# edavalosanaya/FastPoseCNN

Measured on AMD Instinct MI355X. Metric: img/s end-to-end 640x480 inference; hough-vote kernel HBM GB/s vs roofline, higher is better.
Workload: dtype f32

## Files before the change

fastposecnn_amd/_native.py:

```python
import ctypes
import os

import torch

_HERE = os.path.dirname(os.path.abspath(__file__))
LIB_PATH = os.path.join(_HERE, "libfpc_hip.so")

_lib = None

_vp = ctypes.c_void_p
_i = ctypes.c_int
_i64 = ctypes.c_int64
_u64 = ctypes.c_uint64
_f = ctypes.c_float
_d = ctypes.c_double
_sz = ctypes.c_size_t

_SIGNATURES = {
    "fpc_abi_version": (ctypes.c_int, []),
    "fpc_error_string": (ctypes.c_char_p, [_i]),
    "fpc_last_hip_error": (ctypes.c_char_p, []),
    "fpc_generate_hypothesis": (_i, [_vp, _vp, _vp, _vp, _i, _i, _i, _vp]),
    "fpc_voting_for_hypothesis": (_i, [_vp, _vp, _vp, _vp, _i, _i, _i, _f, _vp]),
    "fpc_ransac_workspace_bytes": (_sz, [_i, _i, _i, _i]),
    "fpc_ransac_voting_v3": (_i, [_vp, _vp, _i64, _i64, _i64, _i64, _i, _vp, _i, _i, _i, _vp, _vp, _u64, _f, _i, _i,
                                  _vp, _vp, _vp, _vp, _vp, _vp, _vp, _vp, _vp, _sz, _vp]),
    "fpc_ransac_voting_v3_bits": (_i, [_vp, _vp, _vp, _i64, _i64, _i64, _i64, _i, _vp, _i, _i, _i, _vp, _vp, _u64, _f, _i, _i, _vp, _vp, _vp, _vp, _vp, _vp, _vp, _vp, _vp, _sz, _vp]),
    "fpc_ransac_voting_v3_pose": (_i, [_vp, _vp, _vp, _i64, _i64, _i64, _i64, _i, _vp, _i, _i, _i, _vp, _vp, _u64, _f, _i, _i, _vp, _vp, _vp, _vp, _vp, _vp, _vp, _vp,
                                       _vp, _vp, _vp, _vp, _vp, _vp, _vp, _sz, _vp]),
    "fpc_vote_set_prune": (_i, [_i, _i, ctypes.POINTER(ctypes.c_int32)]),
    "fpc_vote_prune_info": (_i, [_vp, _sz, _i, _i, _i, _i, _vp, _vp]),
    "fpc_class_compress": (_i, [_vp, _vp, _vp, _vp, _vp, _vp, _i, _i, _i, _vp, _vp, _vp, _vp, _vp, _vp]),
    "fpc_class_compress_bits": (_i, [_vp, _vp, _vp, _vp, _vp, _vp, _i, _i, _i, _vp, _vp, _vp, _vp, _vp, _vp, _vp]),
    "fpc_cc_workspace_bytes": (_sz, [_i, _i, _i]),
    "fpc_cc_bits_supported": (_i, [_i, _i, _i]),
    "fpc_fg_bits": (_i, [_vp, _i, _i, _i, _vp, _vp]),
    "fpc_cc_label_bits": (_i, [_vp, _i, _i, _i, _vp, _vp, _vp, _i, _vp, _sz, _vp]),
    "fpc_cc_label": (_i, [_vp, _i, _i, _i, _vp, _vp, _vp, _i, _vp, _sz, _vp]),
    "fpc_aggregate_workspace_bytes": (_sz, [_i]),
    "fpc_aggregate": (_i, [_vp, _vp, _vp, _vp, _vp, _vp, _i, _i, _i, _i, _vp, _vp, _vp, _vp, _vp, _vp, _vp, _vp, _vp, _vp, _sz,
                           _vp]),
    "fpc_aggregate_bits": (_i, [_vp, _vp, _vp, _vp, _vp, _vp, _i, _i, _i, _i, _vp, _vp, _vp, _vp, _vp, _vp, _vp, _vp, _vp, _vp, _vp, _vp, _sz, _vp]),
    "fpc_mask_bits_words": (_sz, [_i, _i]),
    "fpc_pose_errors": (_i, [_vp, _vp, _vp, _vp, _i, _vp, _vp, _vp, _vp, _vp, _vp, _i, _vp, _vp, _vp, _vp]),
    "fpc_pose_metrics_state_words": (_sz, [_i, _i, _i, _i, _i]),
    "fpc_pose_metrics_update": (_i, [_vp, _vp, _vp, _i, _i] + [_vp] * 11 + [_i, _vp, _i, _vp, _i, _vp, _i, _vp, _i, _vp, _i] + [_vp] * 5 + [_i, _vp]),
    "fpc_confusion_update": (_i, [_vp, _vp, _i64, _i, _vp, _vp]),
    "fpc_post_network_backward": (_i, [_vp, _vp, _i, _i, _i, _i, _vp, _vp, _f, _i, _u64, _vp, _vp, _vp, _vp, _vp, _vp]),
    "fpc_vote_refine_backward": (_i, [_vp, _vp, _i64, _i64, _i64, _i64, _i, _i, _i, _vp, _f, _i, _u64, _vp, _vp, _vp]),
    "fpc_class_compress_backward": (_i, [_vp, _vp, _vp, _vp, _vp, _vp, _vp, _i, _i, _i, _vp, _vp, _vp, _vp, _vp]),
    "fpc_mask_losses": (_i, [_vp, _vp, _i, _i, _i, _i64, _i64, _f, _f, _vp, _vp, _vp, _vp]),
    "fpc_match_assign": (_i, [_vp, _vp, _vp, _i, _i, _vp, _vp, _vp, _vp]),
    "fpc_matched_losses": (_i, [_vp, _vp, _vp, _i, _i] + [_vp] * 10 + [_i, _d, _i, _i, _i, ctypes.POINTER(_d)] + [_vp] * 5),
    "fpc_matched_losses_backward": (_i, [_vp, _vp, _vp, _i, _i] + [_vp] * 10 + [_i, _d, _i, _i, _i, ctypes.POINTER(_d)] + [_vp] * 8),
    "fpc_grad_sumsq": (_i, [_vp, _sz, _vp, _vp]),
    "fpc_lookahead_radam_step": (_i, [_vp, _vp, _vp, _vp, _vp, _sz, _f, _f, _f, _f, _f, _i64, _i, _f, _vp, _vp]),
    "fpc_pose_rt": (_i, [_vp, _vp, _vp, _vp, _i, _vp, _vp, _vp, _vp]),
    "fpc_pack_pose_records": (_i, [_vp] * 9 + [_i, _i, _i, _vp, _vp]),
    "fpc_mask_iou_workspace_bytes": (_sz, [_i, _i, _i64]),
    "fpc_mask_iou": (_i, [_vp, _i, _vp, _i, _i64, _i, _vp, _vp, _vp, _vp, _sz, _vp]),
    "fpc_preprocess_workspace_bytes": (_sz, [_i]),
    "fpc_preprocess_u8": (_i, [_vp, _i, _i, _i, ctypes.POINTER(ctypes.c_double), ctypes.POINTER(ctypes.c_double), _i, _vp, _vp,
                               _sz, _vp]),
    "fpc_png_info": (_i, [_vp, _sz, ctypes.POINTER(ctypes.c_int32)]),
    "fpc_png_decode": (_i, [_vp, _sz, _vp, _sz, _i]),
    "fpc_png_decode_batch": (_i, [ctypes.POINTER(_vp), ctypes.POINTER(_sz), _i, _vp, _i, _i, _i]),
    "fpc_gt_build": (_i, [_vp, _i64, _i64, _i, _i, _i, _vp, _vp, _vp, _i, _vp, _vp, _i, _vp, _vp]),
    "fpc_depth_decode": (_i, [_vp, _i, _i, _i, _i, _i, _vp, _vp]),
    "fpc_net_create": (_i, [ctypes.c_char_p, _i, _i, _i, _i, ctypes.POINTER(_vp)]),
    "fpc_net_create_encoder": (_i, [_i, ctypes.POINTER(_i), _i, _i, _i, _i, ctypes.POINTER(_vp)]),
    "fpc_net_destroy": (None, [_vp]),
    "fpc_net_set_graph": (_i, [_vp, _i]),
    "fpc_net_set_split_precision": (_i, [_vp, _i]),
    "fpc_net_param_count": (_i, [_vp]),
    "fpc_net_param_name": (ctypes.c_char_p, [_vp, _i]),
    "fpc_net_param_numel": (_i64, [_vp, _i]),
    "fpc_net_workspace_bytes": (_sz, [_vp]),
    "fpc_net_load_params": (_i, [_vp, _vp, _i, _vp, _sz, _vp]),
    "fpc_net_forward": (_i, [_vp, _vp, _vp, _vp, _vp, _vp, _vp, _vp, _vp, _vp, _vp, _vp, _vp]),
    "fpc_net_forward_bits": (_i, [_vp, _vp, _vp, _vp, _vp, _vp, _vp, _vp, _vp, _vp, _vp, _vp, _vp, _vp]),
    "fpc_net_autotune_next": (_i, [_vp, _i]),
    "fpc_net_conv_count": (_i, [_vp]),
    "fpc_net_conv_plan": (_i, [_vp, _i, ctypes.POINTER(_i)]),
    "fpc_net_copy_plans": (_i, [_vp, _vp]),
    "fpc_net_force_winograd": (_i, [_vp, _i]),
    "fpc_net_force_pointwise": (_i, [_vp, _i]),
    "fpc_net_force_fold": (_i, [_vp, _i]),
    "fpc_net_force_direct_h3": (_i, [_vp, _i]),
    "fpc_net_force_stem_pool": (_i, [_vp, _i]),
    "fpc_act_range": (_i, [_vp, ctypes.c_longlong, _vp, _vp]),
    "fpc_net_survey_next": (_i, [_vp, _vp, _i]),
    "fpc_net_guard_ranges": (_i, [_vp, ctypes.POINTER(ctypes.c_uint32), _i, _f, _f]),
    "fpc_net_guarded": (_i, [_vp, _i]),
    "fpc_stem_pool_tasks": (_i, [_i, _i, ctypes.POINTER(_i64)]),
    "fpc_wino_pack_geometry": (_i, [_i, _i, _i, _i, _i, ctypes.POINTER(_i64)]),
    "fpc_net_set_wino_pack": (_i, [_vp, _i]),
    "fpc_net_set_wino_orient": (_i, [_vp, _i]),
    "fpc_wino_orient_geometry": (_i, [_i, _i, _i, _i, _i, _i, ctypes.POINTER(_i64)]),
    "fpc_net_wino_blocks": (_i64, [_vp]),
    "fpc_net_graph_recorded": (_i, [_vp]),
    "fpc_net_flops": (_i, [_vp, ctypes.POINTER(ctypes.c_double)]),
    "fpc_net_tensor": (_i, [_vp, ctypes.c_char_p, ctypes.POINTER(_vp), ctypes.POINTER(_i), ctypes.POINTER(_i),
                            ctypes.POINTER(_i)]),
    "fpc_conv2d_workspace_bytes": (_sz, [_i, _i, _i, _i, _i, _i, _i]),
    "fpc_conv2d_workspace_bytes_for": (_sz, [_i, _i, _i, _i, _i, _i, _i, _i, _i, _i]),
    "fpc_conv2d_plan": (_i, [_i, _i, _i, _i, _i, _i, _i, _i, _i, _i, ctypes.POINTER(_i)]),
    "fpc_conv2d": (_i, [_vp, _i64, _i64, _i64, _i64, _vp, _vp, _vp, _vp, _vp, _vp, _vp, _i, _i, _i, _i, _i, _i, _i, _i,
                        _i, _i, _i, _i, _i, _vp, _sz, _vp]),
    "fpc_conv2d_wgrad_workspace_bytes": (_sz, [_i, _i, _i, _i, _i, _i, _i]),
    "fpc_upsample_bilinear_fwd": (_i, [_vp, _i64, _i64, _i64, _i64, _vp, _i, _i, _i, _i, _i, _i, _vp]),
    "fpc_upsample_bilinear_bwd_scratch_floats": (_sz, [_i, _i, _i, _i, _i]),
    "fpc_upsample_bilinear_bwd": (_i, [_vp, _i64, _i64, _i64, _i64, _vp, _vp, _i, _i, _i, _i, _i, _i, _vp]),
    "fpc_groupnorm4_relu_scratch_floats": (_sz, [_i, _i, _i]),
    "fpc_groupnorm4_relu_fwd": (_i, [_vp, _vp, _vp, _vp, _vp, _vp, _i, _i, _i, _i, ctypes.c_float, _vp]),
    "fpc_groupnorm4_relu_bwd": (_i, [_vp, _vp, _vp, _vp, _vp, _vp, _vp, _i, _i, _i, _i, _vp]),
    "fpc_batchnorm_scratch_floats": (_sz, [_i, _i]),
    "fpc_batchnorm_fwd": (_i, [_vp, _vp, _vp, _vp, _vp, _vp, _vp, _vp, _vp, _i, _i, _f, _f, _i, _vp]),
    "fpc_batchnorm_bwd": (_i, [_vp, _vp, _vp, _vp, _vp, _vp, _vp, _vp, _vp, _vp, _i, _i, _i, _vp]),
    "fpc_conv2d_wgrad": (_i, [_vp, _i64, _i64, _i64, _vp, _vp, _i, _i, _i, _i, _i, _i, _i, _i, _i, _vp, _sz, _vp]),
    "fpc_conv2d_wgrad_split": (_i, [_vp, _i64, _i64, _i64, _vp, _vp, _i, _i, _i, _i, _i, _i, _i, _i, _i, _vp, _sz, _vp]),
}

EXPORTED = tuple(_SIGNATURES)


def lib():
    global _lib
    if _lib is None:
        if not os.path.exists(LIB_PATH):
            raise RuntimeError(
                f"fastposecnn_amd: {LIB_PATH} is missing — build it with `python -m fastposecnn_amd.build` "
                "(hipcc --offload-arch=gfx950). There is no CPU fallback for the HIP hot path.")
        L = ctypes.CDLL(LIB_PATH)
        for name, (res, args) in _SIGNATURES.items():
            fn = getattr(L, name)
            fn.restype = res
            fn.argtypes = args
        if L.fpc_abi_version() != 11:
            raise RuntimeError("fastposecnn_amd: libfpc_hip.so ABI version mismatch")
        _lib = L
    return _lib


def check(rc, what):
    if rc != 0:
        L = lib()
        msg = L.fpc_error_string(rc).decode()
        hip = L.fpc_last_hip_error().decode() if rc == -3 else ""
        raise RuntimeError(f"fastposecnn_amd: {what} failed: {msg} (code {rc}){' — HIP: ' + hip if hip else ''}")


def ptr(t):
    return None if t is None else t.data_ptr()


_raw_stream = getattr(torch._C, "_cuda_getCurrentRawStream", None)
_cur_device = getattr(torch._C, "_cuda_getDevice", None)


def stream():
    if _raw_stream is not None and _cur_device is not None:
        return _raw_stream(_cur_device())
    return torch.cuda.current_stream().cuda_stream


def require_gpu(*tensors, what="this op"):
    for t in tensors:
        if t is not None and not t.is_cuda:
            raise RuntimeError(f"fastposecnn_amd: {what} runs only on GPU tensors (HIP kernels, no CPU fallback)")


_workspaces = {}


def workspace(tag, device, nbytes):
    key = (tag, device.index, stream())
    ws = _workspaces.get(key)
    if ws is None or ws.numel() < nbytes:
        ws = torch.empty(max(int(nbytes), 256), dtype=torch.uint8, device=device)
        assert ws.data_ptr() % 256 == 0
        _workspaces[key] = ws
    return ws
```

fastposecnn_amd/csrc/net.hip:

```cpp
#include <math.h>
#include <stdio.h>
#include <stdlib.h>
#include <string.h>

#include <initializer_list>
#include <string>
#include <utility>
#include <vector>

#include "net_kernels.hpp"

namespace fpc {

struct PackedConv {
    int Cin = 0, Cinp = 0, Cout = 0, Kh = 1, Kw = 1, stride = 1, pad = 0;
    int Kwp = 1;
    int K = 0, Kpad = 0, Npad = 0;
    int p_w = -1;
    int p_bn = -1;
    int p_bias = -1;
    size_t w_off = 0, scale_off = 0, shift_off = 0;
    size_t wino_off = 0;
    bool wino_ok = false;
    size_t h3_off = 0;
// ... 1118 lines not shown
                        float* logits_xy, float* logits_z, int64_t* cat_mask, float* cq, float* cs, float* cxy, float* cz,
                        uint64_t* fg_bits, fpc_stream_t stream);

extern "C" int fpc_net_forward_bits(fpc_net_t* n, const float* x, float* logits_mask, float* logits_quat,
                                    float* logits_scales, float* logits_xy, float* logits_z, int64_t* cat_mask, float* cq,
                                    float* cs, float* cxy, float* cz, uint64_t* fg_bits, fpc_stream_t stream) {
    const int rc = forward_bits(n, x, logits_mask, logits_quat, logits_scales, logits_xy, logits_z, cat_mask, cq, cs, cxy, cz, fg_bits, stream);
    if (n) n->survey = nullptr;
    return rc;
}

static int forward_bits(fpc_net_t* n, const float* x, float* logits_mask, float* logits_quat, float* logits_scales,
                        float* logits_xy, float* logits_z, int64_t* cat_mask, float* cq, float* cs, float* cxy, float* cz,
                        uint64_t* fg_bits, fpc_stream_t stream) {
    if (!n || !n->loaded || !x || !cat_mask || !cq || !cs || !cxy || !cz) return FPC_EINVAL;
    if (fg_bits && (n->W % 64 != 0 || ((uintptr_t)fg_bits & 7))) return FPC_EINVAL;
    bool any = logits_mask || logits_quat || logits_scales || logits_xy || logits_z;
    bool all = logits_mask && logits_quat && logits_scales && logits_xy && logits_z;
    if (any && !all) return FPC_EINVAL;
    hipStream_t s = (hipStream_t)stream;
    float* ws = n->ws;
    const int B = n->B, H = n->H, W = n->W;

    FPC_TRY(launch_nchw3_to_nhwc4(x, ws + n->a_img4.off, B, H * W, s));
    const bool plain = n->tuning || n->survey;
    if (n->use_graph && !plain && s != nullptr && !n->graph_exec) {
        hipGraph_t g = nullptr;
        if (hipStreamBeginCapture(s, hipStreamCaptureModeThreadLocal) == hipSuccess) {
            int rc = forward_middle(n, s);
            hipError_t e = hipStreamEndCapture(s, &g);
            if (rc) { if (g) (void)hipGraphDestroy(g); return rc; }
            if (e == hipSuccess && g) e = hipGraphInstantiate(&n->graph_exec, g, nullptr, nullptr, 0);
            if (g) (void)hipGraphDestroy(g);
            if (e != hipSuccess) n->graph_exec = nullptr;
        }
        if (!n->graph_exec) { (void)hipGetLastError(); n->use_graph = 0; }
    }
    if (n->use_graph && !plain && s != nullptr && n->graph_exec) {
        if (hipGraphLaunch(n->graph_exec, s) != hipSuccess) return FPC_ELAUNCH;
    } else {
        FPC_TRY(forward_middle(n, s));
    }
    {
        Up4Args u;
        memset(&u, 0, sizeof(u));
        u.lm = ws + n->a_low[0].off; u.lq = ws + n->a_low[1].off; u.lt = ws + n->a_low[2].off; u.ls = ws + n->a_low[3].off;
        u.pm = n->dec[0].head_chp; u.pq = n->dec[1].head_chp; u.pt = n->dec[2].head_chp; u.ps = n->dec[3].head_chp;
        u.o_mask = logits_mask; u.o_quat = logits_quat; u.o_scales = logits_scales; u.o_xy = logits_xy; u.o_z = logits_z;
        u.cat_mask = (long long*)cat_mask; u.cq = cq; u.cs = cs; u.cxy = cxy; u.cz = cz;
        u.B = B; u.hl = n->a_low[0].H; u.wl = n->a_low[0].W; u.H = H; u.W = W; u.C = n->classes;
        u.fg_bits = reinterpret_cast<unsigned long long*>(fg_bits); u.fg_stride = (size_t)((H * W + 4095) / 4096) * 64;
        if (u.hl * 4 != H || u.wl * 4 != W) return FPC_EINVAL;
        FPC_TRY(launch_up4_compress(u, s));
    }
    if (n->tuning) { n->tuning = false; n->tuned = true; }
    return FPC_OK;
}

extern "C" int fpc_net_autotune_next(fpc_net_t* n, int mode) {
    if (!n || !n->loaded || mode < 0 || mode > 2) return FPC_EINVAL;
    n->tuning = true;
    n->tune_mode = mode;
    drop_graph(n);
    return FPC_OK;
}

extern "C" int fpc_net_survey_next(fpc_net_t* n, unsigned* records_dev, int sites) {
    if (n && !records_dev) { n->survey = nullptr; return FPC_OK; }
    if (!n || !n->loaded || ((uintptr_t)records_dev & 3) || sites != (int)n->convs.size()) return FPC_EINVAL;
    n->survey = records_dev;
    return FPC_OK;
}

static ConvPlan range_free_plan(const fpc_net* n, int i) {
    if (n->has_free[i]) return n->free_plan[i];
    const PackedConv& c = n->convs[i];
    ConvPlan q = n->cplan[i];
    if (q.pool) { ConvPlan st; st.stem = 256; return st; }
    if (q.wino) {
        q.wino = wino_form_ok(kWinoW4, c.Cin, c.Cout) ? kWinoW4 : kWinoBf3;
        q.fold = 0;
        return q;
    }
    q.h3 = 0; q.bf3 = 1;
    return q;
}

extern "C" int fpc_net_guard_ranges(fpc_net_t* n, const unsigned* records_host, int sites, float lo, float hi) {
    if (!n || !records_host || sites != (int)n->convs.size() || !(lo >= 0.f) || !(hi > lo)) return FPC_EINVAL;
    auto outside = [&](int site) {
        const unsigned* rec = records_host + 4 * (size_t)site;
        float mx;
        memcpy(&mx, &rec[0], sizeof(mx));
        return rec[2] != 0 && (rec[1] > 0 || mx >= hi || (mx > 0.f && mx < lo));
    };
    int demoted = 0;
    for (int i = 0; i < sites; ++i) {
        if (!n->c_groups[i] || !plan_range_limited(n->cplan[i]) || records_host[4 * (size_t)i + 2] == 0) continue;
        if (!(outside(i) || (n->cplan[i].fold && outside(n->dec[0].lat[3])))) continue;
        n->cplan[i] = range_free_plan(n, i);
        n->guarded[i] = 1;
        ++demoted;
    }
    if (demoted) drop_graph(n);
    return demoted;
}

extern "C" int fpc_net_guarded(const fpc_net_t* n, int i) {
    return n && i >= 0 && i < (int)n->guarded.size() && n->guarded[i] ? 1 : 0;
}

extern "C" int fpc_net_conv_count(const fpc_net_t* n) { return n ? (int)n->convs.size() : 0; }
extern "C" int fpc_net_conv_plan(const fpc_net_t* n, int i, int* out5) {
    if (!n || !out5 || i < 0 || i >= (int)n->convs.size()) return FPC_EINVAL;
    const ConvPlan& p = n->cplan[i];
    out5[0] = p.bm; out5[1] = p.bn;
    if (p.lat) { out5[0] = 128; out5[1] = 32; }
    if (p.stem) { out5[0] = 64; out5[1] = 64; }
    if (p.pw) { out5[0] = pw_tile_pixels(p.pw - 1); out5[1] = 64; }
    out5[2] = encode_plan(p, n->fold_ok && i == n->dec[0].lat[3] && n->cplan[n->dec[0].seg[6]].fold);
    out5[3] = n->convs[i].Cout; out5[4] = n->convs[i].K;
    return FPC_OK;
}

extern "C" int fpc_net_force_winograd(fpc_net_t* n, int form) {
    if (!n || form < 1 || form >= kWinoFormCount) return FPC_EINVAL;
    int changed = 0;
    for (size_t i = 0; i < n->convs.size(); ++i) {
        const PackedConv& c = n->convs[i];
        if (!c.wino_ok || !n->c_groups[i] || !wino_form_ok(form, c.Cin, c.Cout)) continue;
        ConvPlan q = n->cplan[i];
        q.wino = form; q.lat = 0; q.stem = 0;
        if (form != kWinoH3) q.fold = 0;
        n->cplan[i] = q;
        n->guarded[i] = 0;
        ++changed;
    }
    drop_graph(n);
    return changed;
}

extern "C" int fpc_net_force_fold(fpc_net_t* n, int on) {
    if (!n || on < 0 || on > 1 || (on && !n->fold_ok)) return FPC_EINVAL;
    ConvPlan& p = n->cplan[n->dec[0].seg[6]];
    if (p.fold == on) return 0;
    ConvPlan q;
    q.wino = kWinoH3; q.fold = on;
    p = q;
    n->guarded[n->dec[0].seg[6]] = 0;
    drop_graph(n);
    return 1;
}

extern "C" int fpc_net_force_pointwise(fpc_net_t* n, int on) {
    if (!n || on < 0 || on > 1) return FPC_EINVAL;
    int changed = 0;
    for (size_t i = 0; i < n->convs.size(); ++i) {
        const PackedConv& c = n->convs[i];
        if (!n->c_groups[i] || c.Kh != 1 || c.pad != 0 || c.Cinp != c.Cin || c.Cin % 64 || c.Kpad != c.Cin || c.Cout % 64) continue;
        if (on) {
            if (n->cplan[i].pw) continue;
            ConvPlan q;
            q.pw = 1;
            n->cplan[i] = q;
        } else {
            if (!n->cplan[i].pw) continue;
            n->cplan[i] = plan_conv(n->c_howo[i], n->B, c.Cout, c.Kpad / kConvBK, n->c_groups[i]);
        }
        ++changed;
    }
    drop_graph(n);
    return changed;
}

extern "C" int fpc_net_force_direct_h3(fpc_net_t* n, int on) {
    if (!n || on < 0 || on > 1 || (on && !n->h3_packed)) return FPC_EINVAL;
    int changed = 0;
    for (size_t i = 0; i < n->convs.size(); ++i) {
        const PackedConv& c = n->convs[i];
        if (!c.h3_ok || !n->c_groups[i] || on == n->cplan[i].h3) continue;
        const ConvPlan& p = n->cplan[i];
        ConvPlan q = plan_conv(n->c_howo[i], n->B, c.Cout, c.Kpad / kConvBK, n->c_groups[i]);
        if (on && !p.wino && !p.stem && !p.pw) q = p;
        q.bf3 = 0;
        q.h3 = on;
        n->cplan[i] = q;
        n->guarded[i] = 0;
        ++changed;
    }
    drop_graph(n);
    return changed;
}

extern "C" int fpc_net_force_stem_pool(fpc_net_t* n, int on) {
    if (!n || on < 0 || on > 1 || (on && !n->h3_packed)) return FPC_EINVAL;
    if (on && ((n->a_stem.H & 1) || (n->a_stem.W & 63) || (long long)n->H * n->W * 16 >= (1LL << 31))) return FPC_EINVAL;
    ConvPlan& p = n->cplan[n->c_stem];
    if (p.pool == on) return 0;
    ConvPlan q;
    q.stem = 256; q.pool = on;
    p = q;
    n->guarded[n->c_stem] = 0;
    drop_graph(n);
    return 1;
}

extern "C" int fpc_net_copy_plans(fpc_net_t* dst, const fpc_net_t* src) {
    if (!dst || !src || dst->convs.size() != src->convs.size() || dst->H != src->H || dst->W != src->W) return FPC_EINVAL;
    for (size_t i = 0; i < dst->convs.size(); ++i) {
        const PackedConv &a = dst->convs[i], &b = src->convs[i];
        if (a.Cin != b.Cin || a.Cout != b.Cout || a.Kh != b.Kh || a.Kw != b.Kw || a.stride != b.stride || a.Npad != b.Npad ||
            a.Kpad != b.Kpad || dst->c_groups[i] != src->c_groups[i])
            return FPC_EINVAL;
    }
    for (size_t i = 0; i < dst->convs.size(); ++i) {
        const ConvPlan& q = src->cplan[i];
        if (splitk_floats_for(q, dst->c_groups[i] ? dst->c_groups[i] : 1, dst->B, dst->convs[i].Npad) > dst->splitk_floats) continue;
        if (q.nsplit > 1 && q.fused && !can_fuse(q, dst->c_groups[i] ? dst->c_groups[i] : 1, dst->B)) continue;
        if ((q.h3 || q.pool) && !dst->h3_packed) continue;
        dst->cplan[i] = q;
    }
    for (size_t i = 0; i < dst->convs.size(); ++i) {
        const ConvPlan& q = src->free_plan[i];
        const int groups = dst->c_groups[i] ? dst->c_groups[i] : 1;
        dst->has_free[i] = src->has_free[i] && splitk_floats_for(q, groups, dst->B, dst->convs[i].Npad) <= dst->splitk_floats &&
                           !(q.nsplit > 1 && q.fused && !can_fuse(q, groups, dst->B));
        if (dst->has_free[i]) dst->free_plan[i] = q;
        dst->guarded[i] = dst->guarded[i] || src->guarded[i];
        if (dst->guarded[i] && plan_range_limited(dst->cplan[i])) dst->cplan[i] = range_free_plan(dst, (int)i);
    }
    dst->tuned = true;
    drop_graph(dst);
    return FPC_OK;
}

extern "C" int fpc_net_flops(const fpc_net_t* n, double* out3) {
    if (!n || !out3) return FPC_EINVAL;
    double direct = 0.0, executed = 0.0, wino = 0.0;
    for (size_t i = 0; i < n->convs.size(); ++i) {
        if (!n->c_groups[i]) continue;
        const PackedConv& c = n->convs[i];
        const double f = 2.0 * n->B * (double)n->c_howo[i] * c.Cout * c.Cin * c.Kh * c.Kw * n->c_groups[i];
        direct += f;
        if (n->cplan[i].wino) { executed += f / 2.25; wino += f; } else executed += f;
    }
    for (int d = 0; d < 4; ++d)
        direct += 2.0 * n->B * (double)n->a_low[d].H * n->a_low[d].W * 128.0 * n->dec[d].head_ch,
        executed += 2.0 * n->B * (double)n->a_low[d].H * n->a_low[d].W * 128.0 * n->dec[d].head_ch;
    out3[0] = direct; out3[1] = executed; out3[2] = direct > 0.0 ? wino / direct : 0.0;
    return FPC_OK;
}

extern "C" int fpc_net_tensor(const fpc_net_t* n, const char* name, const float** ptr, int* H, int* W, int* C) {
    if (!n || !n->ws || !name || !ptr || !H || !W || !C) return FPC_EINVAL;
    Act t;
    bool ok = false;
    if (!strcmp(name, "stem")) {
        if (n->cplan[n->c_stem].pool) return FPC_EINVAL;
        t = n->a_stem; ok = true;
    }
    else if (!strcmp(name, "pool")) { t = n->a_pool; ok = true; }
    else if (name[0] == 'c' && name[1] >= '2' && name[1] <= '5' && !name[2]) { t = n->a_blk_y[name[1] - '2'].back(); ok = true; }
    else if (name[0] == 'd' && name[1] >= '0' && name[1] <= '3' && name[2] == '.') {
        int d = name[1] - '0';
        const char* r = name + 3;
        if (r[0] == 'p' && r[1] >= '2' && r[1] <= '5' && !r[2]) {
            if (r[1] == '2' && n->cplan[n->dec[0].seg[6]].fold) return FPC_EINVAL;
            t = n->a_p[d]['5' - r[1]]; ok = true;
        }
        else if (!strncmp(r, "seg", 3) && r[3] >= '0' && r[3] <= '6' && !r[4]) { t = n->a_seg[d][r[3] - '0']; ok = true; }
        else if (!strcmp(r, "low")) { t = n->a_low[d]; ok = true; }
    }
    if (!ok) return FPC_EINVAL;
    *ptr = n->ws + t.off; *H = t.H; *W = t.W; *C = t.C;
    return FPC_OK;
}

extern "C" int fpc_stem_pool_tasks(int Ho, int Wo, int64_t* out4) {
    if (!out4 || Ho < 2 || (Ho & 1) || Wo < 64 || (Wo & 63)) return FPC_EINVAL;
    long long o[4];
    stem_pool_tasks(Ho, Wo, kStemPoolBand, o);
    for (int i = 0; i < 4; ++i) out4[i] = o[i];
    return FPC_OK;
}

extern "C" int fpc_wino_pack_geometry(int H, int W, int B, int Cin, int fold, int64_t* out8) {
    if (!out8 || H < 1 || W < 1 || B < 1 || Cin < 1) return FPC_EINVAL;
    const WinoPackGeom q = wino_pack_geometry(H, W, B, Cin, !fold);
    out8[0] = q.G; out8[1] = q.tbx; out8[2] = q.tby; out8[3] = q.patches; out8[4] = q.slots; out8[5] = q.tiles; out8[6] = q.gn_rows;
    out8[7] = q.rx;
    return FPC_OK;
}

extern "C" int fpc_wino_orient_geometry(int H, int W, int B, int Cin, int fold, int pack, int64_t* out9) {
    if (!out9 || H < 1 || W < 1 || B < 1 || Cin < 1) return FPC_EINVAL;
    bool tr;
    const WinoPackGeom q = wino_launch_geometry(H, W, B, Cin, true, pack && !fold, &tr);
    out9[0] = tr ? 1 : 0;
    out9[1] = q.G; out9[2] = q.tbx; out9[3] = q.tby; out9[4] = q.patches; out9[5] = q.slots; out9[6] = q.tiles; out9[7] = q.gn_rows;
    out9[8] = q.rx;
    return FPC_OK;
}

extern "C" size_t fpc_conv2d_workspace_bytes(int B, int Ho, int Wo, int Cin, int Cout, int Kh, int Kw) {
    int K = Cin * Kh * Kw, Kpad = cdiv(K, kConvBK) * kConvBK, Npad = cdiv(Cout, kConvNAlign) * kConvNAlign;
    size_t packed = conv_packed_floats(Npad, Kpad);
    size_t splitk = (size_t)32 * B * (cdiv(Ho * Wo, 128) * 128) * Npad;
    size_t wino = wino_region_floats(kImgH3, Cout, Cin, true);
    return (packed + splitk + wino + kConvTickets) * sizeof(float);
}

namespace {
struct Conv2dLayout { size_t packed, splitk, wino, tickets, total; };
Conv2dLayout conv2d_layout(int B, int Cin, int Cout, int Kh, int Kw, const ConvPlan& p, const Conv2dRequest& r) {
    const int K = Cin * Kh * Kw, Kpad = cdiv(K, kConvBK) * kConvBK, Npad = cdiv(Cout, kConvNAlign) * kConvNAlign;
    Conv2dLayout L;
    L.packed = r.wino ? 0 : conv_packed_floats(Npad, Kpad);
    L.splitk = r.wino ? 0 : (splitk_floats_for(p, 1, B, Npad) + 63) / 64 * 64;
    L.wino = r.wino ? wino_region_floats(kWinoForms[r.wino].image, Cout, Cin, Cout % 128 == 0) : 0;
    L.tickets = (!r.wino && p.fused && p.nsplit > 1) ? kConvTickets : 0;
    L.total = L.packed + L.splitk + L.wino + L.tickets;
    return L;
}
ConvPlan conv2d_plan_for(int B, int Ho, int Wo, int Cin, int Cout, int Kh, int Kw, int bm, int bn, const Conv2dRequest& r) {
    const int Kpad = cdiv(Cin * Kh * Kw, kConvBK) * kConvBK;
    ConvPlan p = plan_conv(Ho * Wo, B, Cout, Kpad / kConvBK, 1, r.wino ? 0 : bm, bn, r.wino ? 1 : r.nsplit);
    p.bf3 = r.bf3 ? 1 : 0;
    p.h3 = r.h3 ? 1 : 0;
    if (r.two_launch) p.fused = 0;
    p.lat = r.lat;
    p.stem = r.stem ? 256 : 0;
    p.pool = r.pool ? 1 : 0;
    p.pw = r.pw;
    p.wino = r.wino;
    return p;
}
}

extern "C" int fpc_conv2d_plan(int B, int Ho, int Wo, int Cin, int Cout, int Kh, int Kw, int bm, int bn, int nsplit,
                               int* out4) {
    if (!out4) return FPC_EINVAL;
    const int Kpad = cdiv(Cin * Kh * Kw, kConvBK) * kConvBK;
    const Conv2dRequest r = decode_plan(nsplit);
    ConvPlan p = plan_conv(Ho * Wo, B, Cout, Kpad / kConvBK, 1, bm, bn, r.nsplit);
    p.wino = r.wino;
    out4[0] = p.bm; out4[1] = p.bn; out4[2] = r.wino ? nsplit : p.nsplit; out4[3] = plan_gn_rows(p, Ho, Wo, B, Cin, r.pack, r.orient);
    return FPC_OK;
}

extern "C" size_t fpc_conv2d_workspace_bytes_for(int B, int Ho, int Wo, int Cin, int Cout, int Kh, int Kw, int bm, int bn,
                                                 int nsplit) {
    if (B < 1 || Ho < 1 || Wo < 1 || Cin < 1 || Cout < 1 || Kh < 1 || Kw < 1) return 0;
    const Conv2dRequest r = decode_plan(nsplit);
    const ConvPlan p = conv2d_plan_for(B, Ho, Wo, Cin, Cout, Kh, Kw, bm, bn, r);
    return std::max<size_t>(conv2d_layout(B, Cin, Cout, Kh, Kw, p, r).total * sizeof(float), 256);
}

extern "C" int fpc_conv2d(const float* in, int64_t sb, int64_t sh, int64_t sw, int64_t sc, const float* w_oihw,
                          const float* scale, const float* shift, const float* res, const float* up, float* out,
                          float* gn_part, int B, int Hi, int Wi, int Cin, int Cout, int Kh, int Kw, int stride, int pad,
                          int relu, int bm, int bn, int nsplit, void* ws, size_t ws_bytes, fpc_stream_t stream) {
    if (!in || !w_oihw || !out || !ws || B < 1 || Kh != Kw) return FPC_EINVAL;
    int Ho = conv_out(Hi, Kh, stride, pad), Wo = conv_out(Wi, Kw, stride, pad);
    if (Ho < 1 || Wo < 1) return FPC_EINVAL;
    const Conv2dRequest rq = decode_plan(nsplit);
    const int wino = rq.wino;
    ConvPlan p = conv2d_plan_for(B, Ho, Wo, Cin, Cout, Kh, Kw, bm, bn, rq);
    const Conv2dLayout lay = conv2d_layout(B, Cin, Cout, Kh, Kw, p, rq);
    if (ws_bytes < lay.total * sizeof(float) || ((uintptr_t)ws & 255)) return FPC_EWORKSPACE;
    PackedConv c;
    c.Cin = c.Cinp = Cin; c.Cout = Cout; c.Kh = Kh; c.Kw = Kw; c.stride = stride; c.pad = pad;
    c.K = Cin * Kh * Kw; c.Kpad = cdiv(c.K, kConvBK) * kConvBK; c.Npad = cdiv(Cout, kConvNAlign) * kConvNAlign;
    hipStream_t s = (hipStream_t)stream;
    float* packed = (float*)ws;
    if (rq.stem) {
        if (Cin != 4 || Kh != 7 || stride != 2 || pad != 3 || Cout != 64 || sc != 1 || sw != 4 || sh != (int64_t)4 * Wi ||
            sb != (int64_t)4 * Hi * Wi || res || up || gn_part)
            return FPC_EINVAL;
        c.Kwp = 8; c.K = 4 * 7 * 8; c.Kpad = 224;
        FPC_TRY((rq.pool ? launch_pack_weight_h3 : launch_pack_weight_bf3)(w_oihw, packed, Cout, Cin, Cin, Kh, Kw, c.Kwp, c.Npad, c.Kpad, s));
        fpc_net tmp0;
        tmp0.B = B; tmp0.ws = packed; tmp0.splitk_off = lay.packed;
        ConvArgs a0;
        fill_conv_args(&tmp0, a0, c, p, Hi, Wi, Ho, Wo, sb, sh, sw, sc, relu != 0, 0);
        a0.Cin = 8 * c.Cinp; a0.Kw = 1; a0.K = c.K; a0.lanepx = 1;
        a0.p[0] = ConvPtrs{in, packed, out, scale, shift, nullptr, nullptr, nullptr};
        return rq.pool ? launch_stem_pool(a0, packed, out, Ho / 2, Wo / 2, s) : launch_conv_plan(a0, p, 1, s);
    }
    static_assert(FPC_IGEMM_DMA_B, "the split-precision direct form stages its B rows from the bf16 planes by LDS-DMA; a build that loads "
                                   "them from the f32 image must pack that image here as well");
    if (!wino) FPC_TRY((p.h3 ? launch_pack_weight_h3 : p.bf3 ? launch_pack_weight_bf3 : launch_pack_weight)(w_oihw, packed, Cout, Cin, Cin, Kh, Kw, Kw, c.Npad, c.Kpad, s));
    int mode = (sc == 1 && Cin % kConvBK == 0 && Kh * Kw <= 32 && ((int64_t)Hi + 2 * pad) * sh * 4 < ((int64_t)1 << 31)) ? 0
               : (sc == 1 && Cin % 4 == 0 && sw % 4 == 0 && sh % 4 == 0 && sb % 4 == 0 && ((uintptr_t)in & 15) == 0) ? 2 : 1;
    fpc_net tmp;
    tmp.B = B;
    tmp.wino_pack = rq.pack ? 1 : 0;
    tmp.wino_orient = rq.orient ? 1 : 0;
    tmp.ws = packed;
    tmp.splitk_off = lay.packed;
    ConvArgs a;
    fill_conv_args(&tmp, a, c, p, Hi, Wi, Ho, Wo, sb, sh, sw, sc, relu != 0, mode);
    a.p[0] = ConvPtrs{in, packed, out, scale, shift, res, up, gn_part};
    a.zeros = nullptr;
    a.tickets = nullptr;
    if (lay.tickets) {
        float* tk = packed + lay.packed + lay.splitk + lay.wino;
        a.tickets = (int*)tk;
        if (hipMemsetAsync(tk, 0, kConvTickets * sizeof(int), s) != hipSuccess) return FPC_ELAUNCH;
    }
#ifdef FPC_STAMP_WINO
    if (wino && relu == 77) { a.dbg = gn_part; a.p[0].gn_part = nullptr; a.relu = 0; }
#endif
#ifdef FPC_STAMP_IGEMM
    if (!wino && relu == 77) { a.dbg = gn_part; a.p[0].gn_part = nullptr; a.relu = 0; }
#endif
    if (wino) {
        if (Kh != 3 || stride != 1 || pad != 1 || Cin % 8 || Cout % 64 || sc != 1 || up || sw != Cin ||
            sh != (int64_t)Wi * Cin || sb != (int64_t)Hi * Wi * Cin)
            return FPC_EINVAL;
        float* wp = packed + lay.packed + lay.splitk;
        if (!wino_form_ok(wino, Cin, Cout)) return FPC_EINVAL;
        const WinoImage img = kWinoForms[wino].image;
        if (rq.orient && wino_orient_rule(Ho, Wo)) FPC_TRY(launch_wino_pack_h3(w_oihw, wp + wino_image_offset(img, Cout, Cin), Cout, Cin, true, s));
        else FPC_TRY(kWinoImages[img].pack(w_oihw, wp + wino_image_offset(img, Cout, Cin), Cout, Cin, s));
        a.wino_w[0] = wp;
        a.zeros = zero_page();
        if (!a.zeros) {
            float* zp = wp + lay.wino - 64;
            if (hipMemsetAsync(zp, 0, 64 * sizeof(float), s) != hipSuccess) return FPC_ELAUNCH;
            a.zeros = zp;
        }
        return launch_conv_plan(a, p, 1, s);
    }
    if (p.h3) {
        if (mode != 0) return FPC_EINVAL;
        a.h3_w[0] = packed;
        return launch_conv_plan(a, p, 1, s);
    }
    a.bf3 = (p.bf3 && mode == 0) ? 1 : 0;
    if (p.bf3 && mode != 0) return FPC_EINVAL;
    if (p.lat || p.pw) return launch_conv_plan(a, p, 1, s);
    return run_conv(nullptr, a, 1, 0, s);
}
```

fastposecnn_amd/csrc/net_kernels.hpp:

```cpp
#pragma once
#include "common.hpp"

namespace fpc {

#ifndef FPC_IGEMM_DMA_B
#define FPC_IGEMM_DMA_B 1
#endif

constexpr int kMaxGroup = 4;
constexpr int kConvBK = 32;
constexpr int kConvNAlign = 128;
constexpr int kConvTickets = 16384;

struct ConvPtrs {
    const float* in;
    const float* w;
    float* out;
    const float* scale;
    const float* shift;
    const float* res;
    const float* up;
    float* gn_part;
};

struct ConvArgs {
    ConvPtrs p[kMaxGroup];
    float* splitk_ws;
    int* tickets;
    int fused;
    int B, Hi, Wi, Cin, Ho, Wo, Cout, Npad, Kh, Kw, stride, pad, K, Kpad;
    long long in_sb, in_sh, in_sw, in_sc;
    int relu, nsplit, mtiles, ntiles, ksteps, bm, bn, generic, groups;
    int bf3;
    int h3;
    int lanepx;
    const float* wino_w[kMaxGroup];
    const float* h3_w[kMaxGroup];
    const float* zeros;
    const float* fold_in;
    const float* fold_w[kMaxGroup];
    const float* fold_w2[kMaxGroup];
    const float* fold_up[kMaxGroup];
    const float* fold_tab[kMaxGroup];
    int fold_cin;
    float fold_lat_ms;
    void* dbg;
    long long wino_blocks;
    int wino_pack;
    int wino_orient;
};

struct LatArgs {
    const float* in;
    const unsigned short* wpl[kMaxGroup];
    float* out[kMaxGroup];
    const float* shift[kMaxGroup];
    const float* up[kMaxGroup];
    int B, Ho, Wo, Cout, Npad, Kpad, groups, relu;
    unsigned bias_mask;
    int parts;
    int h3;
};
int launch_lateral1x1(const LatArgs& a, hipStream_t s);

struct PwArgs {
    const float* in;
    const unsigned short* wpl[kMaxGroup];
    float* out[kMaxGroup];
    const float* scale[kMaxGroup];
    const float* shift[kMaxGroup];
    const float* res[kMaxGroup];
    const float* up[kMaxGroup];
    long long in_sb, in_sh, in_sw;
    int B, Ho, Wo, Cin, Cout, Npad, Kpad, stride, groups, relu;
    int has_scale, has_shift, has_res, has_up;
    int variant;
};
int launch_conv1x1(const PwArgs& a, hipStream_t s);
inline int pw_tile_pixels(int variant) { return variant == 0 ? 64 : 128; }

struct StemArgs {
    const float* in;
    const unsigned short* wpl;
    float* out;
    const float* scale;
    const float* shift;
    int B, Hi, Wi, Ho, Wo, Cout, Npad, Kpad, relu;
    int grid;
};
int launch_stem7x7(const StemArgs& a, hipStream_t s);

struct StemPoolArgs {
    const float* in;
    const unsigned short* wpl;
    float* out;
    const float* scale;
    const float* shift;
    int B, Hi, Wi, Ho, Wo, Hp, Wp, Npad, Kpad, relu;
    int band;
    int grid;
};
constexpr int kStemPoolBand = 10;
int launch_stem_pool_h3(const StemPoolArgs& a, hipStream_t s);
void stem_pool_tasks(int Ho, int Wo, int band, long long out4[4]);

constexpr int kMaxGnSites = 4;
struct GnFinArgs {
    const float* gn_part[kMaxGnSites * kMaxGroup];
    const float* gamma[kMaxGnSites * kMaxGroup];
    const float* beta[kMaxGnSites * kMaxGroup];
    float* affine[kMaxGnSites * kMaxGroup];
    int P[kMaxGnSites];
    long long count[kMaxGnSites];
    int B, C, groups, sites;
    float eps;
};

constexpr int kMaxUpJobs = 2;
struct GnUpArgs {
    const float* in[kMaxUpJobs * kMaxGroup];
    const float* affine[kMaxUpJobs * kMaxGroup];
    float* out[kMaxUpJobs * kMaxGroup];
    int h[kMaxUpJobs], w[kMaxUpJobs];
    int B, C, jobs;
};

struct MergeHeadArgs {
    const float* t_lo[kMaxGroup][3];
    const float* a_lo[kMaxGroup][3];
    const float* t_hi[kMaxGroup];
    const float* a_hi[kMaxGroup];
    const float* hw[kMaxGroup];
    const float* hb[kMaxGroup];
    float* out[kMaxGroup];
    int ch[kMaxGroup];
    int chp[kMaxGroup];
    int B, h, w, C;
};

struct HeadPartArgs {
    const float* t[kMaxGroup][3];
    const float* aff[kMaxGroup][3];
    const float* hw[kMaxGroup];
    const float* hb[kMaxGroup];
    const float* lsum[kMaxGroup];
    float* out[kMaxGroup];
    int ch[kMaxGroup], chp[kMaxGroup];
    int B, H, W, C, hl, wl;
};
int launch_head_part(const HeadPartArgs& a, bool hi, int groups, hipStream_t s);

struct Up4Args {
    const float* lm; const float* lq; const float* lt; const float* ls;
    int pm, pq, pt, ps;
    float* o_mask; float* o_quat; float* o_scales; float* o_xy; float* o_z;
    long long* cat_mask; float* cq; float* cs; float* cxy; float* cz;
    int B, hl, wl, H, W, C;
    unsigned long long* fg_bits; size_t fg_stride;
};

#ifdef FPC_STAMP_WINO
constexpr bool kWinoStamp = true;
#else
constexpr bool kWinoStamp = false;
#endif

struct WinoArgs {
    ConvPtrs p[kMaxGroup];
    long long* dbg;
    const float* zeros;
    int variant;
    int groups;
    int waves;
    int B, H, W, Cin, Cout, relu, tbx, tby;
    const float* in2[kMaxGroup];
    const float* w2[kMaxGroup];
    const float* btab[kMaxGroup];
    int fold, Cin2;
    int pack, pack_rx;
    int orient;
};
int launch_conv_wino(const WinoArgs& a, int groups, hipStream_t s);
const float* zero_page();
int launch_wino_pack(const float* w_oihw, float* packed, int Cout, int Cin, hipStream_t s);
int launch_wino_pack_bf3(const float* w_oihw, float* packed, int Cout, int Cin, hipStream_t s);
int launch_conv_wino_c128(const WinoArgs& a, int groups, hipStream_t s);
int launch_wino_pack_c128(const float* w_oihw, float* packed, int Cout, int Cin, hipStream_t s);
int launch_conv_wino_w4(const WinoArgs& a, int groups, hipStream_t s);
int launch_conv_wino_h2(const WinoArgs& a, int groups, hipStream_t s);
int launch_wino_pack_h2(const float* w_oihw, float* packed, int Cout, int Cin, hipStream_t s);
int launch_absmax_bits(const float* w, long long n, unsigned* out_bits, hipStream_t s);
int launch_act_range(const float* x, long long n, unsigned* rec4, hipStream_t s);
int launch_conv_wino_h3(const WinoArgs& a, int groups, hipStream_t s);
struct WinoPackGeom { int G, tbx, tby, rx; long long patches, slots, tiles; int gn_rows; };
WinoPackGeom wino_pack_geometry(int H, int W, int B, int Cin, bool allow);
bool wino_orient_rule(int H, int W);
WinoPackGeom wino_launch_geometry(int H, int W, int B, int Cin, bool orient, bool pack_allow, bool* transposed);
int launch_wino_pack_h3(const float* w_oihw, float* packed, int Cout, int Cin, bool transpose, hipStream_t s);
int launch_wino_pack_h3_pair(const float* w1, float* packed1, int Cin1, const float* w2, float* packed2, int Cin2, int Cout, bool transpose,
                             hipStream_t s);
int launch_fold_compose(const float* W, const float* L, const float* bias, float* wc, float* btab, int Cout, int Cmid, int Cin,
                        bool transpose, hipStream_t s);
int launch_conv(const ConvArgs& a, int groups, hipStream_t s);
int launch_conv_splitk_epilogue(const ConvArgs& a, int groups, hipStream_t s);
int launch_maxpool3x3s2(const float* in, float* out, int B, int Hi, int Wi, int C, int Ho, int Wo, hipStream_t s);
int launch_gn_finalize(const GnFinArgs& a, int groups, hipStream_t s);
int launch_gn_relu_up2(const GnUpArgs& a, int groups, hipStream_t s);
int launch_merge_head(const MergeHeadArgs& a, int groups, hipStream_t s);
int launch_up4_compress(const Up4Args& a, hipStream_t s);
void launch_up4_compress7x4(const Up4Args& a, hipStream_t s);

struct Lerp { int i0, i1; float l0, l1; };
__device__ __forceinline__ Lerp lerp_coord(int dst, int in, int out) {
    float scale = out > 1 ? (float)(in - 1) / (float)(out - 1) : 0.f;
    float src = scale * (float)dst;
    Lerp L;
    L.i0 = (int)src;
    L.i1 = L.i0 + (L.i0 < in - 1 ? 1 : 0);
    L.l1 = src - (float)L.i0;
    L.l0 = 1.f - L.l1;
    return L;
}

__device__ __forceinline__ Lerp lerp_scaled(int dst, int in, float scale) {
    float src = scale * (float)dst;
    Lerp L;
    L.i0 = (int)src;
    L.i1 = L.i0 + (L.i0 < in - 1 ? 1 : 0);
    L.l1 = src - (float)L.i0;
    L.l0 = 1.f - L.l1;
    return L;
}

int launch_pack_weight(const float* w_oihw, float* packed, int Cout, int Cin, int Cinp, int Kh, int Kw, int Kwp, int Npad,
                       int Kpad, hipStream_t s);
int launch_pack_weight_bf3(const float* w_oihw, float* packed, int Cout, int Cin, int Cinp, int Kh, int Kw, int Kwp, int Npad,
                           int Kpad, hipStream_t s);
inline size_t conv_packed_floats(int Npad, int Kpad) { return ((size_t)Npad * Kpad * 5 / 2 + 63) / 64 * 64; }
int launch_pack_weight_h3(const float* w_oihw, float* packed, int Cout, int Cin, int Cinp, int Kh, int Kw, int Kwp, int Npad,
                          int Kpad, hipStream_t s);
inline size_t h3_packed_floats(int Npad, int Kpad) { return ((size_t)Npad * Kpad + 2 + 63) / 64 * 64; }
int launch_nchw3_to_nhwc4(const float* x, float* out, int B, int HW, hipStream_t s);
int launch_fold_bn(const float* gamma, const float* beta, const float* mean, const float* var, float eps, int C,
                   float* scale, float* shift, hipStream_t s);

}
```

fastposecnn_amd/csrc/wino_h2.hip:

```cpp
#include <algorithm>
#ifdef FPC_STAMP_WINO
#include <cstdlib>
#endif
#include "wino_tile.hpp"

namespace fpc {
using namespace wino_tile;

namespace {
constexpr int kStepBytes = 16 * 64 * 32;
static_assert(kLdsFloats >= 2 * kInFloats, "the K loop's two input buffers live in the output image's space");
}

template <int MODE>
__global__ __launch_bounds__(256, 1) void k_conv_wino_h2(const WinoArgs a) {
    __shared__ __attribute__((aligned(16))) float lds[kLdsFloats];
    long long* const dbg = kWinoStamp ? a.dbg : nullptr;
    const long long t_entry = dbg ? clock64() : 0;
    const int t = threadIdx.x, lane = t & 63;
    const int wi = __builtin_amdgcn_readfirstlane(t >> 6);
    const int li = lane & 31, lh = lane >> 5;
    const int H = a.H, W = a.W, Cin = a.Cin, Cout = a.Cout, HW = H * W;
    const int nkb = Cin >> 3;
    const WinoPatch pt = wino_patch<false>(blockIdx.x, Cout / kBN, a.groups, a.tbx, a.tby, 0, W, a.B);
    const int nb = pt.nb, nnb = Cout / kBN;
    const ConvPtrs P = wino_group(a.p[0], a.p[1], a.p[2], a.p[3], pt.grp);
    const int y_in0 = 2 * pt.ty0 - 1, x_in0 = 2 * pt.tx0 - 1;

    f32x16 acc[4][2][2];
    const __amdgpu_buffer_rsrc_t rs_w = make_rsrc(reinterpret_cast<const char*>(P.w) + (size_t)nb * nkb * kStepBytes);
    const float inv_s = P.w[(size_t)nnb * nkb * (kStepBytes / 4)];
    const int vo_u = lane * 16;
    int so_u = wi * 4 * 2048;
    u32x4 U[4][2];
#define FPC_H2_LOAD_U(J, NT) U[J][NT] = __builtin_bit_cast(u32x4, __builtin_amdgcn_raw_buffer_load_b128(rs_w, vo_u, so_u + (J) * 2048 + (NT) * 1024, 0))
#pragma unroll
    for (int j = 0; j < 4; ++j)
#pragma unroll
        for (int nt = 0; nt < 2; ++nt) FPC_H2_LOAD_U(j, nt);
    if (nkb > 1) so_u += kStepBytes;
    const float* isb = P.in + (size_t)pt.b * HW * Cin;
    unsigned ivo[5];
    unsigned long long imask[5];
    wino_stage_plan<false>(ivo, imask, wi, lane, y_in0, x_in0, H, W, Cin, 0, pt.pk_ks, pt.pk_two);
#define FPC_H2_ISSUE_IN(BUF) wino_issue_in(lds + (BUF) * kInFloats, wi, ivo, imask, isb)
    int in_a[2], in_b[2];
    const float sgn = wino_frag<false>(in_a, in_b, wi, li, lh, pt.pk_ks);
    wino_zero_ring(lds, t, 2, y_in0, x_in0, H, W, false);
    FPC_H2_ISSUE_IN(0);
    if (nkb > 1) isb += 8;
    FPC_H2_ISSUE_IN(1);
    if (nkb > 2) isb += 8;
#pragma unroll
    for (int j = 0; j < 4; ++j)
#pragma unroll
        for (int mt = 0; mt < 2; ++mt)
#pragma unroll
            for (int nt = 0; nt < 2; ++nt)
#pragma unroll
                for (int r = 0; r < 16; ++r) acc[j][mt][nt][r] = 0.f;

    const long long t_issued = dbg ? clock64() : 0;
    asm volatile("s_waitcnt vmcnt(0)" ::: "memory");
    const long long t_landed = dbg ? clock64() : 0;
    __syncthreads();
    const long long t_synced = dbg ? clock64() : 0;

    u32x4 TA1[4][2], TA2[4][2];
    f32x4 vn[2][4];
#define FPC_H2_SPLIT_PAIR(J, MT, PAIR)                                                                        \
    do {                                                                                                      \
        const float x0_ = vn[MT][J][2 * (PAIR)], x1_ = vn[MT][J][2 * (PAIR) + 1];                             \
        const fp16x2 h_ = __builtin_amdgcn_cvt_pkrtz(x0_, x1_);                                               \
        const float r0_ = x0_ - (float)h_[0], r1_ = x1_ - (float)h_[1];                                       \
        const unsigned k1_ = __builtin_bit_cast(unsigned, h_);                                                \
        const unsigned k2_ = __builtin_bit_cast(unsigned, __builtin_amdgcn_cvt_pkrtz(r0_, r1_));              \
        asm volatile("" :: "v"(k1_), "v"(k2_));                                                               \
        TA1[J][MT][PAIR] = k1_; TA1[J][MT][2 + (PAIR)] = k1_; TA2[J][MT][PAIR] = k2_; TA2[J][MT][2 + (PAIR)] = k2_; \
    } while (0)
#pragma unroll
    for (int j = 0; j < 4; ++j)
#pragma unroll
        for (int mt = 0; mt < 2; ++mt) { TA1[j][mt] = u32x4{0u, 0u, 0u, 0u}; TA2[j][mt] = u32x4{0u, 0u, 0u, 0u}; }
    {
#pragma unroll
        for (int mt = 0; mt < 2; ++mt) {
            f32x4 e[4];
#pragma unroll
            for (int c = 0; c < 4; ++c)
                e[c] = fma_s4(sgn, *reinterpret_cast<const f32x4*>(lds + in_b[c >> 1] + (c & 1) * in_cs + mt * in_ms),
                              *reinterpret_cast<const f32x4*>(lds + in_a[c >> 1] + (c & 1) * in_cs + mt * in_ms));
            vn[mt][0] = sub_s4(e[0], e[2]); vn[mt][1] = add_s4(e[1], e[2]); vn[mt][2] = sub_s4(e[2], e[1]); vn[mt][3] = sub_s4(e[1], e[3]);
#pragma unroll
            for (int j = 0; j < 3; ++j) { FPC_H2_SPLIT_PAIR(j, mt, 0); FPC_H2_SPLIT_PAIR(j, mt, 1); }
        }
    }
    __syncthreads();

#define FPC_H2_MFMA(J, MT, NT, A, B) acc[J][MT][NT] = __builtin_amdgcn_mfma_f32_32x32x16_f16(__builtin_bit_cast(f16x8, A), __builtin_bit_cast(f16x8, B), acc[J][MT][NT], 0, 0, 0)
#define FPC_H2_PIN4(V) asm volatile("" :: "v"(V))
    int cur = 0;
    const long long c_begin = dbg ? clock64() : 0, r_begin = dbg ? wall_clock64() : 0;
#pragma unroll 1
    for (int kb = 0; kb < nkb; ++kb) {
        if (!(MODE & 2) && !(MODE & 8)) FPC_H2_ISSUE_IN(cur);
        const float* In = lds + (cur ^ 1) * kInFloats;
        f32x4 da[2][4], db[2][4], e[2][4];
        __builtin_amdgcn_s_setprio(1);
#define FPC_H2_SPLIT_Q(J, Q) do { if ((Q) == 0) FPC_H2_SPLIT_PAIR(J, 0, 0); if ((Q) == 1) FPC_H2_SPLIT_PAIR(J, 0, 1); if ((Q) == 2) FPC_H2_SPLIT_PAIR(J, 1, 0); if ((Q) == 3) FPC_H2_SPLIT_PAIR(J, 1, 1); } while (0)
#pragma unroll
        for (int j = 0; j < 4; ++j)
#pragma unroll
            for (int g = 0; g < 2; ++g)
#pragma unroll
                for (int mt = 0; mt < 2; ++mt)
#pragma unroll
                    for (int nt = 0; nt < 2; ++nt) {
                        const int sl = 8 * j + 4 * g + 2 * mt + nt;
                        if (g == 0) FPC_H2_MFMA(j, mt, nt, TA1[j][mt], U[j][nt]);
                        if (g == 1) {
                            FPC_H2_MFMA(j, mt, nt, TA2[j][mt], U[j][nt]);
                            if (mt == 1 && !(MODE & 1)) FPC_H2_LOAD_U(j, nt);
                        }
                        if (sl < 4) {
#pragma unroll
                            for (int c = 2 * (sl & 1); c < 2 * (sl & 1) + 2; ++c) {
                                da[sl >> 1][c] = *reinterpret_cast<const f32x4*>(In + in_a[c >> 1] + (c & 1) * in_cs + (sl >> 1) * in_ms);
                                db[sl >> 1][c] = *reinterpret_cast<const f32x4*>(In + in_b[c >> 1] + (c & 1) * in_cs + (sl >> 1) * in_ms);
                            }
                            FPC_H2_SPLIT_Q(3, sl);
                        }
                        if (sl >= 4 && sl < 12) {
                            const int m_ = (sl - 4) >> 2, c = (sl - 4) & 3;
                            e[m_][c] = fma_s4(sgn, db[m_][c], da[m_][c]);
                            FPC_H2_PIN4(e[m_][c]);
                        }
                        if (sl >= 12 && sl < 20) {
                            const int m_ = (sl - 12) >> 2, jx = (sl - 12) & 3;
                            if (jx == 0) vn[m_][0] = sub_s4(e[m_][0], e[m_][2]);
                            if (jx == 1) vn[m_][1] = add_s4(e[m_][1], e[m_][2]);
                            if (jx == 2) vn[m_][2] = sub_s4(e[m_][2], e[m_][1]);
                            if (jx == 3) vn[m_][3] = sub_s4(e[m_][1], e[m_][3]);
                            FPC_H2_PIN4(vn[m_][jx]);
                        }
                        if (sl >= 20 && sl < 24) FPC_H2_SPLIT_Q(0, sl - 20);
                        if (sl >= 24 && sl < 28) FPC_H2_SPLIT_Q(1, sl - 24);
                        if (sl >= 28) FPC_H2_SPLIT_Q(2, sl - 28);
                        __builtin_amdgcn_sched_barrier(0);
                    }
#undef FPC_H2_SPLIT_Q
        __builtin_amdgcn_s_setprio(0);
        so_u += kb + 2 < nkb ? kStepBytes : 0;
        isb += kb + 3 < nkb ? 8 : 0;
        if (!(MODE & 2)) {
            if (MODE & 1) asm volatile("s_waitcnt vmcnt(0)" ::: "memory");
            else asm volatile("s_waitcnt vmcnt(8)" ::: "memory");
            if (!(MODE & 4)) __syncthreads();
        }
        cur ^= 1;
    }
#undef FPC_H2_MFMA
#undef FPC_H2_SPLIT_PAIR
#undef FPC_H2_PIN4
#undef FPC_H2_ISSUE_IN
#undef FPC_H2_LOAD_U
    asm volatile("s_waitcnt vmcnt(0)" ::: "memory");
    const long long t_kend = dbg ? clock64() : 0;
    if (dbg && lane == 0) {
        long long* o = dbg + ((size_t)blockIdx.x * 4 + wi) * 8;
        o[0] = t_issued - t_entry; o[1] = t_landed - t_issued; o[2] = t_synced - t_landed;
        o[3] = t_kend - c_begin; o[4] = wall_clock64() - r_begin; o[5] = nkb; o[6] = c_begin - t_entry;
    }
    wino_output<false, false>(lds, acc, P, pt, WinoEpi{H, W, Cout, a.relu, a.tbx, a.tby, 0}, inv_s, nullptr, dbg, t_kend, t, wi);
}

__global__ __launch_bounds__(256) void k_absmax_bits(const float* __restrict__ w, long long n, unsigned* __restrict__ out) {
    __shared__ unsigned s_m[4];
    unsigned m = 0u;
    const long long n4 = n >> 2;
    for (long long g = (long long)blockIdx.x * blockDim.x + threadIdx.x; g < n4; g += (long long)gridDim.x * blockDim.x) {
        const f32x4 v = reinterpret_cast<const f32x4*>(w)[g];
        m = max(max(m, __builtin_bit_cast(unsigned, fabsf(v[0]))), max(__builtin_bit_cast(unsigned, fabsf(v[1])),
                max(__builtin_bit_cast(unsigned, fabsf(v[2])), __builtin_bit_cast(unsigned, fabsf(v[3])))));
    }
    if (blockIdx.x == 0)
        for (long long g = 4 * n4 + threadIdx.x; g < n; g += blockDim.x) m = max(m, __builtin_bit_cast(unsigned, fabsf(w[g])));
#pragma unroll
    for (int o = 32; o > 0; o >>= 1) m = max(m, (unsigned)__shfl_xor((int)m, o, 64));
    if ((threadIdx.x & 63) == 0) s_m[threadIdx.x >> 6] = m;
    __syncthreads();
    if (threadIdx.x == 0) {
        m = max(max(s_m[0], s_m[1]), max(s_m[2], s_m[3]));
        if (m) atomicMax(out, m);
    }
}

int launch_absmax_bits(const float* w, long long n, unsigned* out, hipStream_t s) {
    hipLaunchKernelGGL(k_absmax_bits, dim3((unsigned)std::min<long long>((n / 4 + 255) / 256 + 1, 64)), dim3(256), 0, s, w, n, out);
    return check_launch();
}

template <bool PAIR>
__global__ __launch_bounds__(256) void k_wino_pack_fp16(const float* __restrict__ w, unsigned short* __restrict__ out, float* __restrict__ tail,
                                                        int Cout, int Cin, int tr) {
    const float wmax = __builtin_bit_cast(float, reinterpret_cast<const unsigned*>(tail)[1]);
    int ex = 0;
    if (wmax > 0.f && wmax < 3.0e38f) { (void)frexpf(2.25f * wmax, &ex); ex = 13 - ex; }
    ex = max(-100, min(100, ex));
    const float sc = ldexpf(1.0f, ex);
    if (blockIdx.x == 0 && threadIdx.x == 0) tail[0] = ldexpf(1.0f, -ex);
    const long long total = (long long)Cout * Cin;
    for (long long g = (long long)blockIdx.x * blockDim.x + threadIdx.x; g < total; g += (long long)gridDim.x * blockDim.x) {
        const int ci = (int)(g % Cin), co = (int)(g / Cin);
        const float* k = w + ((size_t)co * Cin + ci) * 9;
        float gg[4][3];
        const int sr = tr ? 1 : 3, scol = tr ? 3 : 1;
#pragma unroll
        for (int c = 0; c < 3; ++c) {
            const float g0 = k[c * scol] * sc, g1 = k[sr + c * scol] * sc, g2 = k[2 * sr + c * scol] * sc;
            gg[0][c] = g0;
            gg[1][c] = 0.5f * (g0 + g1 + g2);
            gg[2][c] = 0.5f * (g0 - g1 + g2);
            gg[3][c] = g2;
        }
        const int nb = co >> 6, col = co & 63, nt = col >> 5, kb = ci >> 3, cil = ci & 7, e = cil & 3;
        const int ln = (cil >> 2) * 32 + (col & 31);
        unsigned short* img = out + (PAIR ? ((size_t)nb * (Cin >> 4) + (kb >> 1)) * (kPairBytes / 2) : ((size_t)nb * (Cin >> 3) + kb) * (kStepBytes / 2));
        const int f0 = PAIR ? (nt * 2048 + ln * 16) / 2 + (kb & 1) * 4 + e : (nt * 1024 + ln * 16) / 2 + e;
        constexpr int xi_s = PAIR ? 4096 / 2 : 2048 / 2, p2 = PAIR ? 512 : 4;
#pragma unroll
        for (int i = 0; i < 4; ++i) {
            const float r0 = gg[i][0], r1 = gg[i][1], r2 = gg[i][2];
            const float u[4] = {r0, 0.5f * (r0 + r1 + r2), 0.5f * (r0 - r1 + r2), r2};
#pragma unroll
            for (int jx = 0; jx < 4; ++jx) {
                const float x = u[jx];
                const fp16x2 h = __builtin_amdgcn_cvt_pkrtz(x, 0.f);
                const float r = x - (float)h[0];
                const fp16x2 h2 = __builtin_amdgcn_cvt_pkrtz(r, 0.f);
                unsigned short* frag = img + (4 * i + jx) * xi_s + f0;
                frag[0] = (unsigned short)(__builtin_bit_cast(unsigned, h) & 0xFFFFu);
                frag[p2] = (unsigned short)(__builtin_bit_cast(unsigned, h2) & 0xFFFFu);
            }
        }
    }
}

int launch_wino_pack_fp16(const float* w_oihw, float* packed, int Cout, int Cin, bool pair, const float* w_also, int Cin_also, bool transpose,
                          hipStream_t s) {
    if (Cin % (pair ? 16 : 8) != 0 || Cout % kBN != 0 || ((uintptr_t)w_oihw & 15) || ((uintptr_t)w_also & 15)) return FPC_EINVAL;
    float* tail = packed + (size_t)16 * Cout * Cin;
    if (hipMemsetAsync(tail, 0, 2 * sizeof(float), s) != hipSuccess) return FPC_ELAUNCH;
    int rc = launch_absmax_bits(w_oihw, (long long)Cout * Cin * 9, reinterpret_cast<unsigned*>(tail) + 1, s);
    if (!rc && w_also) rc = launch_absmax_bits(w_also, (long long)Cout * Cin_also * 9, reinterpret_cast<unsigned*>(tail) + 1, s);
    if (rc) return rc;
    const dim3 grid((unsigned)std::min<long long>(((long long)Cout * Cin + 255) / 256, 4096));
    if (pair) hipLaunchKernelGGL(k_wino_pack_fp16<true>, grid, dim3(256), 0, s, w_oihw, reinterpret_cast<unsigned short*>(packed), tail, Cout, Cin, transpose ? 1 : 0);
    else hipLaunchKernelGGL(k_wino_pack_fp16<false>, grid, dim3(256), 0, s, w_oihw, reinterpret_cast<unsigned short*>(packed), tail, Cout, Cin, transpose ? 1 : 0);
    return check_launch();
}

int launch_wino_pack_h2(const float* w_oihw, float* packed, int Cout, int Cin, hipStream_t s) {
    return launch_wino_pack_fp16(w_oihw, packed, Cout, Cin, false, nullptr, 0, false, s);
}

int launch_conv_wino_h2(const WinoArgs& a, int groups, hipStream_t s) {
    long long nblk;
    if (const int rc = wino_tile_check(a, groups, 8, kStepBytes, false, &nblk)) return rc;
#ifdef FPC_STAMP_WINO
    static const int mode = getenv("FPC_H2_MODE") ? atoi(getenv("FPC_H2_MODE")) : 0;
    if (mode == 1) hipLaunchKernelGGL(k_conv_wino_h2<1>, dim3((unsigned)nblk), dim3(256), 0, s, a);
    else if (mode == 2) hipLaunchKernelGGL(k_conv_wino_h2<2>, dim3((unsigned)nblk), dim3(256), 0, s, a);
    else if (mode == 3) hipLaunchKernelGGL(k_conv_wino_h2<3>, dim3((unsigned)nblk), dim3(256), 0, s, a);
    else if (mode == 5) hipLaunchKernelGGL(k_conv_wino_h2<5>, dim3((unsigned)nblk), dim3(256), 0, s, a);
    else if (mode == 9) hipLaunchKernelGGL(k_conv_wino_h2<9>, dim3((unsigned)nblk), dim3(256), 0, s, a);
    else if (mode == 4) hipLaunchKernelGGL(k_conv_wino_h2<4>, dim3((unsigned)nblk), dim3(256), 0, s, a);
    else
#endif
    hipLaunchKernelGGL(k_conv_wino_h2<0>, dim3((unsigned)nblk), dim3(256), 0, s, a);
    return check_launch();
}

}
```

fastposecnn_amd/csrc/wino_h3.hip:

```cpp
#include <algorithm>
#ifdef FPC_STAMP_WINO
#include <cstdlib>
#endif
#include <type_traits>
#include "wino_tile.hpp"

namespace fpc {
using namespace wino_tile;

namespace {

constexpr int kRing = 4;
static_assert(kLdsFloats >= kRing * kInFloats, "the K loop's input ring lives in the output image's space");

__device__ __forceinline__ const float* sgpr_ptr(const float* p) {
    const unsigned long long v = reinterpret_cast<unsigned long long>(p);
    const unsigned lo = __builtin_amdgcn_readfirstlane((unsigned)v), hi = __builtin_amdgcn_readfirstlane((unsigned)(v >> 32));
    return reinterpret_cast<const float*>(((unsigned long long)hi << 32) | lo);
}

}

template <int VAR, bool FOLD, bool PACK, bool TR = false>
__global__ __launch_bounds__(256, 1) void k_conv_wino_h3(const WinoArgs a) {
    __shared__ __attribute__((aligned(16))) float lds[kLdsFloats];
    long long* const dbg = kWinoStamp ? a.dbg : nullptr;
    const long long t_entry = dbg ? clock64() : 0;
    const int t = threadIdx.x, lane = t & 63;
    const int wi = __builtin_amdgcn_readfirstlane(t >> 6);
    const int li = lane & 31, lh = lane >> 5;
    const int H = a.H, W = a.W, Cout = a.Cout;
    const int nnb = Cout / kBN;
    const WinoPatch pt = wino_patch<PACK>(blockIdx.x, nnb, a.groups, a.tbx, a.tby, a.pack, W, a.B);
    const int nb = pt.nb, grp = pt.grp, pk_ks = pt.pk_ks;
    const ConvPtrs P = wino_group(a.p[0], a.p[1], a.p[2], a.p[3], grp);
    const int y_in0 = 2 * pt.ty0 - 1, x_in0 = 2 * pt.tx0 - 1;

    f32x16 acc[4][2][2];
    float inv_s = 1.f;
    long long t_issued = 0, t_landed = 0, t_synced = 0, c_begin = 0, r_begin = 0;
    const bool stamp = dbg != nullptr;

    auto kloop = [&](auto ph, const float* src, const float* wimg, const int Cs, const int up) __attribute__((always_inline)) {
    constexpr int PH = decltype(ph)::value;
    constexpr bool SKIPC = PH == 1;
    const int nkb = Cs >> 3;
    const int npair = nkb >> 1;
    const __amdgpu_buffer_rsrc_t rs_w = make_rsrc(reinterpret_cast<const char*>(wimg) + (size_t)nb * npair * kPairBytes);
    inv_s = wimg[(size_t)nnb * npair * (kPairBytes / 4)];
    const int vo_u = lane * 16;
    int so_u = wi * 4 * 4096;
    u32x4 U1[4][2], U2[4][2];
#define FPC_H3_XI_LIVE(J) (!(SKIPC && (J) == 2))
#define FPC_H3_LOAD_U1_AT(SO, J, NT) do { if (FPC_H3_XI_LIVE(J)) U1[J][NT] = __builtin_bit_cast(u32x4, __builtin_amdgcn_raw_buffer_load_b128(rs_w, vo_u, (SO) + (J) * 4096 + (NT) * 2048, 0)); } while (0)
#define FPC_H3_LOAD_U2_AT(SO, J, NT) do { if (FPC_H3_XI_LIVE(J)) U2[J][NT] = __builtin_bit_cast(u32x4, __builtin_amdgcn_raw_buffer_load_b128(rs_w, vo_u, (SO) + (J) * 4096 + (NT) * 2048 + 1024, 0)); } while (0)
#define FPC_H3_LOAD_U1(J, NT) FPC_H3_LOAD_U1_AT(so_u, J, NT)
#define FPC_H3_LOAD_U2(J, NT) FPC_H3_LOAD_U2_AT(so_u, J, NT)
#pragma unroll
    for (int j = 0; j < 4; ++j)
#pragma unroll
        for (int nt = 0; nt < 2; ++nt) { FPC_H3_LOAD_U1(j, nt); FPC_H3_LOAD_U2(j, nt); }
    if (npair > 1) so_u += kPairBytes;

    const float* isb = sgpr_ptr(src + (size_t)pt.b * (H >> up) * (W >> up) * Cs);
    unsigned ivo[5];
    unsigned long long imask[5];
    wino_stage_plan<PACK, TR>(ivo, imask, wi, lane, y_in0, x_in0, H, W, Cs, up, pk_ks, pt.pk_two);
#define FPC_H3_ISSUE_IN(BUF, PTR) wino_issue_in(lds + (BUF) * kInFloats, wi, ivo, imask, PTR)
    int in_a[2], in_b[2];
    const float sgn = wino_frag<PACK>(in_a, in_b, wi, li, lh, pk_ks);
    wino_zero_ring(lds, t, kRing, y_in0, x_in0, H, W, PACK && pk_ks < kTX);
    FPC_H3_ISSUE_IN(0, isb);
    isb += 8;
    FPC_H3_ISSUE_IN(1, isb);
    isb += 8;
    FPC_H3_ISSUE_IN(2, nkb > 2 ? isb : isb - 8);
    isb += 8;
    int sn = 3;
#pragma unroll
    for (int j = 0; j < 4; ++j)
#pragma unroll
        for (int mt = 0; mt < 2; ++mt)
#pragma unroll
            for (int nt = 0; nt < 2; ++nt)
#pragma unroll
                for (int r = 0; r < 16; ++r)
                    if (PH == 0) acc[j][mt][nt][r] = 0.f;

    t_issued = stamp ? clock64() : 0;
    asm volatile("s_waitcnt vmcnt(10)" ::: "memory");
    t_landed = stamp ? clock64() : 0;
    __syncthreads();
    t_synced = stamp ? clock64() : 0;

    u32x4 TA1[4][2], TA2[4][2];
    f32x4 vn[2][4];
    float m1;
    asm volatile("s_mov_b32 %0, 0xbf800000" : "=s"(m1));
#define FPC_H3_SPLIT_PAIR(J, MT, PAIR, HALF) FPC_H3_SPLIT_PAIR_V(vn, J, MT, PAIR, HALF)
#define FPC_H3_SPLIT_PAIR_V(V, J, MT, PAIR, HALF)                                                             \
    if (FPC_H3_XI_LIVE(J)) do {                                                                               \
        const float x0_ = V[MT][J][2 * (PAIR)], x1_ = V[MT][J][2 * (PAIR) + 1];                               \
        const fp16x2 h_ = __builtin_amdgcn_cvt_pkrtz(x0_, x1_);                                               \
                                                          \
        const float r0_ = VAR == 1 ? x0_ - (float)h_[0] : __builtin_fmaf((float)h_[0], m1, x0_);              \
        const float r1_ = VAR == 1 ? x1_ - (float)h_[1] : __builtin_fmaf((float)h_[1], m1, x1_);              \
        const unsigned k1_ = __builtin_bit_cast(unsigned, h_);                                                \
        const unsigned k2_ = __builtin_bit_cast(unsigned, __builtin_amdgcn_cvt_pkrtz(r0_, r1_));              \
        asm volatile("" :: "v"(k1_), "v"(k2_));                                                               \
        TA1[J][MT][2 * (HALF) + (PAIR)] = k1_; TA2[J][MT][2 * (HALF) + (PAIR)] = k2_;                         \
    } while (0)
#pragma unroll
    for (int j = 0; j < 4; ++j)
#pragma unroll
        for (int mt = 0; mt < 2; ++mt) { TA1[j][mt] = u32x4{0u, 0u, 0u, 0u}; TA2[j][mt] = u32x4{0u, 0u, 0u, 0u}; }
    {
#pragma unroll
        for (int mt = 0; mt < 2; ++mt) {
            f32x4 e[4];
#pragma unroll
            for (int c = 0; c < 4; ++c)
                e[c] = fma_s4(sgn, *reinterpret_cast<const f32x4*>(lds + in_b[c >> 1] + (c & 1) * in_cs + mt * in_ms),
                              *reinterpret_cast<const f32x4*>(lds + in_a[c >> 1] + (c & 1) * in_cs + mt * in_ms));
            vn[mt][0] = sub_s4(e[0], e[2]); vn[mt][1] = add_s4(e[1], e[2]); vn[mt][2] = sub_s4(e[2], e[1]); vn[mt][3] = sub_s4(e[1], e[3]);
#pragma unroll
            for (int j = 0; j < 3; ++j) { FPC_H3_SPLIT_PAIR(j, mt, 0, 0); FPC_H3_SPLIT_PAIR(j, mt, 1, 0); }
        }
    }
    asm volatile("s_waitcnt vmcnt(0)" ::: "memory");
    __syncthreads();

#define FPC_H3_MFMA(J, MT, NT, A, B) do { if (FPC_H3_XI_LIVE(J)) acc[J][MT][NT] = __builtin_amdgcn_mfma_f32_32x32x16_f16(__builtin_bit_cast(f16x8, A), __builtin_bit_cast(f16x8, B), acc[J][MT][NT], 0, 0, 0); } while (0)
#define FPC_H3_PIN4(V) asm volatile("" :: "v"(V))
#define FPC_H3_SPLIT_Q(J, Q, HALF) do { if ((Q) == 0) FPC_H3_SPLIT_PAIR(J, 0, 0, HALF); if ((Q) == 1) FPC_H3_SPLIT_PAIR(J, 0, 1, HALF); if ((Q) == 2) FPC_H3_SPLIT_PAIR(J, 1, 0, HALF); if ((Q) == 3) FPC_H3_SPLIT_PAIR(J, 1, 1, HALF); } while (0)
    c_begin = stamp ? clock64() : 0; r_begin = stamp ? wall_clock64() : 0;
#pragma unroll 1
    for (int p = 0; p < npair; ++p) {
        {
            const float* InE = lds + ((2 * p + 1) & 3) * kInFloats;
            f32x4 ea[2][4], eb[2][4];
#pragma unroll
            for (int mt = 0; mt < 2; ++mt)
#pragma unroll
                for (int c = 0; c < 4; ++c) {
                    ea[mt][c] = *reinterpret_cast<const f32x4*>(InE + in_a[c >> 1] + (c & 1) * in_cs + mt * in_ms);
                    eb[mt][c] = *reinterpret_cast<const f32x4*>(InE + in_b[c >> 1] + (c & 1) * in_cs + mt * in_ms);
                }
            __builtin_amdgcn_sched_barrier(0);
            if (sn < nkb) { FPC_H3_ISSUE_IN((sn & 3), isb); isb += 8; }
            if (sn + 1 < nkb) { FPC_H3_ISSUE_IN(((sn + 1) & 3), isb); isb += 8; }
            sn += 2;
#pragma unroll
            for (int q = 0; q < 4; ++q) FPC_H3_SPLIT_Q(3, q, 0);
            __builtin_amdgcn_sched_barrier(0);
#pragma unroll
            for (int mt = 0; mt < 2; ++mt) {
                f32x4 e[4];
#pragma unroll
                for (int c = 0; c < 4; ++c) e[c] = fma_s4(sgn, eb[mt][c], ea[mt][c]);
                vn[mt][0] = sub_s4(e[0], e[2]); vn[mt][1] = add_s4(e[1], e[2]); vn[mt][2] = sub_s4(e[2], e[1]); vn[mt][3] = sub_s4(e[1], e[3]);
                FPC_H3_SPLIT_PAIR(0, mt, 0, 1); FPC_H3_SPLIT_PAIR(0, mt, 1, 1);
            }
        }
        __builtin_amdgcn_sched_barrier(0);
        const float* In = lds + ((2 * p + 2) & 3) * kInFloats;
        f32x4 da[2][4], db[2][4], e[2][4];
        __builtin_amdgcn_s_setprio(1);
#pragma unroll
        for (int j = 0; j < 4; ++j)
#pragma unroll
            for (int g = 0; g < 3; ++g)
#pragma unroll
                for (int mt = 0; mt < 2; ++mt)
#pragma unroll
                    for (int nt = 0; nt < 2; ++nt) {
                        const int sl = 12 * j + 4 * g + 2 * mt + nt;
                        if (g == 0) FPC_H3_MFMA(j, mt, nt, TA1[j][mt], U1[j][nt]);
                        if (g == 1) {
                            FPC_H3_MFMA(j, mt, nt, TA2[j][mt], U1[j][nt]);
                            if (mt == 1) FPC_H3_LOAD_U1(j, nt);
                        }
                        if (g == 2) {
                            FPC_H3_MFMA(j, mt, nt, TA1[j][mt], U2[j][nt]);
                            if (mt == 1) FPC_H3_LOAD_U2(j, nt);
                        }
                        if (sl < 4) {
#pragma unroll
                            for (int c = 2 * (sl & 1); c < 2 * (sl & 1) + 2; ++c) {
                                da[sl >> 1][c] = *reinterpret_cast<const f32x4*>(In + in_a[c >> 1] + (c & 1) * in_cs + (sl >> 1) * in_ms);
                                db[sl >> 1][c] = *reinterpret_cast<const f32x4*>(In + in_b[c >> 1] + (c & 1) * in_cs + (sl >> 1) * in_ms);
                            }
                        }
                        if (sl >= 4 && sl < 12) {
                            const int m_ = (sl - 4) >> 2, c = (sl - 4) & 3;
                            e[m_][c] = fma_s4(sgn, db[m_][c], da[m_][c]);
                            FPC_H3_PIN4(e[m_][c]);
                        }
                        if (sl < 4) FPC_H3_SPLIT_Q(1, sl, 1);
                        if (sl >= 4 && sl < 8) FPC_H3_SPLIT_Q(2, sl - 4, 1);
                        if (sl >= 8 && sl < 12) FPC_H3_SPLIT_Q(3, sl - 8, 1);
                        if (sl >= 12 && sl < 20 && !(SKIPC && ((sl - 12) & 3) == 2)) {
                            const int m_ = (sl - 12) >> 2, jx = (sl - 12) & 3;
                            if (jx == 0) vn[m_][0] = sub_s4(e[m_][0], e[m_][2]);
                            if (jx == 1) vn[m_][1] = add_s4(e[m_][1], e[m_][2]);
                            if (jx == 2) vn[m_][2] = sub_s4(e[m_][2], e[m_][1]);
                            if (jx == 3) vn[m_][3] = sub_s4(e[m_][1], e[m_][3]);
                            FPC_H3_PIN4(vn[m_][jx]);
                        }
                        if (sl >= 20 && sl < 24) FPC_H3_SPLIT_Q(0, sl - 20, 0);
                        if (sl >= 24 && sl < 28) FPC_H3_SPLIT_Q(1, sl - 24, 0);
                        if (sl >= 36 && sl < 40) FPC_H3_SPLIT_Q(2, sl - 36, 0);
                        __builtin_amdgcn_sched_barrier(0);
                    }
        __builtin_amdgcn_s_setprio(0);
        so_u += p + 2 < npair ? kPairBytes : 0;
        if (PH == 0) asm volatile("s_waitcnt vmcnt(16)" ::: "memory");
        if (PH == 1) asm volatile("s_waitcnt vmcnt(12)" ::: "memory");
        __syncthreads();
    }
#undef FPC_H3_MFMA
#undef FPC_H3_SPLIT_PAIR
#undef FPC_H3_SPLIT_PAIR_V
#undef FPC_H3_SPLIT_Q
#undef FPC_H3_PIN4
#undef FPC_H3_ISSUE_IN
#undef FPC_H3_LOAD_U1
#undef FPC_H3_LOAD_U2
#undef FPC_H3_LOAD_U1_AT
#undef FPC_H3_LOAD_U2_AT
#undef FPC_H3_XI_LIVE
    };

    if (!FOLD) {
        kloop(std::integral_constant<int, 0>(), P.in, P.w, a.Cin, 0);
    } else {
        kloop(std::integral_constant<int, 0>(), P.in, P.w, a.Cin, 0);
        kloop(std::integral_constant<int, 1>(), wino_group(a.in2[0], a.in2[1], a.in2[2], a.in2[3], grp), wino_group(a.w2[0], a.w2[1], a.w2[2], a.w2[3], grp), a.Cin2, 1);
    }
    const long long t_kend = dbg ? clock64() : 0;
    if (!(FOLD && PACK) && dbg && lane == 0) {
        long long* o = dbg + ((size_t)blockIdx.x * 4 + wi) * 8;
        o[0] = t_issued - t_entry; o[1] = t_landed - t_issued; o[2] = t_synced - t_landed;
        o[3] = t_kend - c_begin; o[4] = wall_clock64() - r_begin; o[5] = a.Cin >> 3; o[6] = c_begin - t_entry;
    }
    wino_output<PACK, FOLD, TR>(lds, acc, P, pt, WinoEpi{H, W, Cout, a.relu, a.tbx, a.tby, a.pack_rx}, inv_s,
                            wino_group(a.btab[0], a.btab[1], a.btab[2], a.btab[3], grp), dbg, t_kend, t, wi);
}

WinoPackGeom wino_pack_geometry(int H, int W, int B, int Cin, bool allow) {
    WinoPackGeom q;
    const int tcw = cdiv(W, 2), tch = cdiv(H, 2);
    q.G = 1;
    q.tby = cdiv(tch, kTY);
    if (allow && tcw >= kTX && 2LL * H * W * Cin * (long long)sizeof(float) < (1LL << 32)) {
        int best = cdiv(tcw, kTX);
        for (int g = 2; g <= std::min(B, 8); ++g)
            if ((long long)cdiv(g * tcw, kTX) * q.G < (long long)best * g) { best = cdiv(g * tcw, kTX); q.G = g; }
    }
    q.tbx = cdiv(q.G * tcw, kTX);
    q.rx = 1;
    for (int f = 0; f < q.G; ++f) q.rx = std::max(q.rx, (f * tcw + tcw - 1) / kTX - (f * tcw) / kTX + 1);
    q.patches = (long long)q.tby * ((long long)(B / q.G) * q.tbx + cdiv((B % q.G) * tcw, kTX));
    q.slots = q.patches * kNT;
    q.tiles = (long long)B * tch * tcw;
    q.gn_rows = q.tby * q.rx;
    return q;
}

static int wino_fold_check(const WinoArgs& a, int groups) {
    if (a.Cin2 % 16 != 0 || (a.H | a.W) & 1 || (long long)(a.H / 2) * (a.W / 2) * a.Cin2 * (long long)sizeof(float) >= (1LL << 32) ||
        (long long)(a.Cin2 >> 4) * kPairBytes >= (1LL << 31) || a.relu || a.dbg)
        return FPC_EINVAL;
    for (int g = 0; g < groups; ++g)
        if (!a.in2[g] || !a.w2[g] || !a.btab[g] || a.p[g].scale || a.p[g].shift || a.p[g].res || a.p[g].up) return FPC_EINVAL;
    return 0;
}

bool wino_orient_rule(int H, int W) {
    const int tcw = cdiv(W, 2), tch = cdiv(H, 2);
    return tcw % kTX == 0 && tch % kTY != 0 && tch >= kTY;
}

WinoPackGeom wino_launch_geometry(int H, int W, int B, int Cin, bool orient, bool pack_allow, bool* transposed) {
#ifdef FPC_STAMP_WINO
    static const bool g1 = getenv("FPC_H3_ORIENT_G1") && atoi(getenv("FPC_H3_ORIENT_G1")) != 0;
#else
    constexpr bool g1 = false;
#endif
    *transposed = orient && wino_orient_rule(H, W);
    return *transposed ? wino_pack_geometry(W, H, B, Cin, !g1) : wino_pack_geometry(H, W, B, Cin, pack_allow);
}

int launch_conv_wino_h3(const WinoArgs& a, int groups, hipStream_t s) {
    long long nblk;
    if (a.orient) {
        WinoArgs t = a;
        std::swap(t.H, t.W);
        if (a.pack < 1 || a.dbg) return FPC_EINVAL;
        if (const int rc = wino_tile_check(t, groups, 16, kPairBytes, true, &nblk)) return rc;
        if (a.fold) {
            if (const int rc = wino_fold_check(a, groups)) return rc;
            hipLaunchKernelGGL((k_conv_wino_h3<0, true, true, true>), dim3((unsigned)nblk), dim3(256), 0, s, t);
        } else {
            hipLaunchKernelGGL((k_conv_wino_h3<0, false, true, true>), dim3((unsigned)nblk), dim3(256), 0, s, t);
        }
        return check_launch();
    }
    if (const int rc = wino_tile_check(a, groups, 16, kPairBytes, a.pack > 1, &nblk)) return rc;
    if (a.pack > 1) {
        hipLaunchKernelGGL((k_conv_wino_h3<0, false, true>), dim3((unsigned)nblk), dim3(256), 0, s, a);
        return check_launch();
    }
    if (a.fold) {
        if (const int rc = wino_fold_check(a, groups)) return rc;
        hipLaunchKernelGGL((k_conv_wino_h3<0, true, false>), dim3((unsigned)nblk), dim3(256), 0, s, a);
        return check_launch();
    }
#ifdef FPC_STAMP_WINO
    static const int var = getenv("FPC_H3_VAR") ? atoi(getenv("FPC_H3_VAR")) : 0;
    if (var == 1) hipLaunchKernelGGL((k_conv_wino_h3<1, false, false>), dim3((unsigned)nblk), dim3(256), 0, s, a);
    else
#endif
    hipLaunchKernelGGL((k_conv_wino_h3<0, false, false>), dim3((unsigned)nblk), dim3(256), 0, s, a);
    return check_launch();
}

__global__ __launch_bounds__(256) void k_fold_compose(const float* __restrict__ w, const float* __restrict__ l, const float* __restrict__ bias,
                                                      float* __restrict__ wc, float* __restrict__ btab, int Cout, int Cmid, int Cin, int tr) {
    const int g = blockIdx.x * blockDim.x + threadIdx.x;
    const int nw = Cout * Cin * 9;
    if (g < nw) {
        const int tap = g % 9, k = (g / 9) % Cin, o = g / (9 * Cin);
        double acc = 0.0;
        for (int c = 0; c < Cmid; ++c) acc += (double)w[((size_t)o * Cmid + c) * 9 + tap] * (double)l[(size_t)c * Cin + k];
        wc[g] = (float)acc;
    } else if (g < nw + 16 * Cout) {
        const int o = (g - nw) % Cout, cls = (g - nw) / Cout, rc = cls >> 2, cc = cls & 3;
        double acc = 0.0;
        for (int ky = (rc & 1); ky < 3 - ((rc >> 1) & 1); ++ky)
            for (int kx = (cc & 1); kx < 3 - ((cc >> 1) & 1); ++kx)
                for (int c = 0; c < Cmid; ++c) acc += (double)w[((size_t)o * Cmid + c) * 9 + (tr ? kx * 3 + ky : ky * 3 + kx)] * (double)bias[c];
        btab[(size_t)cls * Cout + o] = (float)acc;
    }
}

int launch_fold_compose(const float* W, const float* L, const float* bias, float* wc, float* btab, int Cout, int Cmid, int Cin,
                        bool transpose, hipStream_t s) {
    if (!W || !L || !bias || !wc || !btab || Cout < 1 || Cmid < 1 || Cin < 1) return FPC_EINVAL;
    const long long work = (long long)Cout * Cin * 9 + 16LL * Cout;
    hipLaunchKernelGGL(k_fold_compose, dim3((unsigned)((work + 255) / 256)), dim3(256), 0, s, W, L, bias, wc, btab, Cout, Cmid, Cin, transpose ? 1 : 0);
    return check_launch();
}

int launch_wino_pack_h3_pair(const float* w1, float* packed1, int Cin1, const float* w2, float* packed2, int Cin2, int Cout, bool transpose,
                             hipStream_t s) {
    if (Cin2 % 16 != 0 || ((uintptr_t)w2 & 15)) return FPC_EINVAL;
    const int rc = launch_wino_pack_fp16(w1, packed1, Cout, Cin1, true, w2, Cin2, transpose, s);
    return rc ? rc : launch_wino_pack_fp16(w2, packed2, Cout, Cin2, true, w1, Cin1, transpose, s);
}

int launch_wino_pack_h3(const float* w_oihw, float* packed, int Cout, int Cin, bool transpose, hipStream_t s) {
    return launch_wino_pack_fp16(w_oihw, packed, Cout, Cin, true, nullptr, 0, transpose, s);
}

}
```

fastposecnn_amd/csrc/wino_tile.hpp:

```cpp
#pragma once
#include <algorithm>
#include "net_kernels.hpp"

namespace fpc {
namespace wino_tile {

typedef float f32x16 __attribute__((ext_vector_type(16)));
typedef unsigned u32x4 __attribute__((ext_vector_type(4)));
typedef _Float16 f16x8 __attribute__((ext_vector_type(8)));
typedef __fp16 fp16x2 __attribute__((ext_vector_type(2)));

constexpr int kTX = 8, kTY = 8;
constexpr int kRW = 2 * kTX + 2, kRH = 2 * kTY + 2;
constexpr int kBN = 64;
constexpr int kNT = kTX * kTY;
constexpr int kInPieces = 18;
constexpr int kInFloats = kInPieces * 256;
constexpr int kPairBytes = 16 * 2 * 2 * 64 * 16;
constexpr int kLdsFloats = 4 * 2 * kNT * kBN;

__device__ __forceinline__ __amdgpu_buffer_rsrc_t make_rsrc(const void* base) {
    return __builtin_amdgcn_make_buffer_rsrc(const_cast<void*>(base), 0, 0x7FFFFFFF, 0x00020000);
}
__device__ __forceinline__ f32x4 fma_s4(float s, f32x4 b, f32x4 a) {
    return f32x4{__builtin_fmaf(s, b[0], a[0]), __builtin_fmaf(s, b[1], a[1]), __builtin_fmaf(s, b[2], a[2]), __builtin_fmaf(s, b[3], a[3])};
}
__device__ __forceinline__ f32x4 sub_s4(f32x4 a, f32x4 b) { return f32x4{a[0] - b[0], a[1] - b[1], a[2] - b[2], a[3] - b[3]}; }
__device__ __forceinline__ f32x4 add_s4(f32x4 a, f32x4 b) { return f32x4{a[0] + b[0], a[1] + b[1], a[2] + b[2], a[3] + b[3]}; }

__device__ __forceinline__ unsigned lds_addr(const void* p) { return (unsigned)(size_t)(__attribute__((address_space(3))) const void*)p; }

struct WinoPatch {
    int nb, grp, bx, by, b, tx0, ty0;
    int pk_ks, pk_raw, pk_slot;
    bool pk_two;
};
template <bool PACK>
__device__ __forceinline__ WinoPatch wino_patch(int bid, int nnb, int groups, int tbx, int tby, int pack, int W, int B) {
    WinoPatch q;
    q.pk_ks = 99; q.pk_raw = 99; q.pk_slot = 0; q.pk_two = false;
    q.nb = bid % nnb; bid /= nnb;
    q.grp = bid % groups; bid /= groups;
    if constexpr (!PACK) {
        q.bx = bid % tbx; bid /= tbx;
        q.by = bid % tby;
        q.b = bid / tby;
        q.tx0 = q.bx * kTX;
    } else {
        const int G = pack, tcw = (W + 1) >> 1, per = tbx * tby;
        const int g = bid / per, rem = bid - g * per;
        const int nf = min(G, B - g * G);
        const int tbxg = min(tbx, (nf * tcw + kTX - 1) / kTX);
        q.bx = rem % tbxg; q.by = rem / tbxg;
        const int f = (kTX * q.bx) / tcw;
        q.tx0 = kTX * q.bx - f * tcw;
        q.b = g * G + f;
        q.pk_raw = tcw - q.tx0;
        q.pk_ks = q.pk_raw < kTX ? q.pk_raw : 99;
        q.pk_two = q.pk_ks < kTX && f + 1 < nf;
        q.pk_slot = q.bx - (f * tcw) / kTX;
    }
    q.ty0 = q.by * kTY;
    return q;
}
template <class T>
__device__ __forceinline__ T wino_group(const T v0, const T v1, const T v2, const T v3, int grp) {
    T r = v0;
    if (grp == 1) r = v1;
    if (grp == 2) r = v2;
    if (grp == 3) r = v3;
    return r;
}

template <bool PACK, bool TR = false>
__device__ __forceinline__ void wino_stage_plan(unsigned (&ivo)[5], unsigned long long (&imask)[5], int wi, int lane, int y_in0, int x_in0, int H,
                                                int W, int Cs, int up, int pk_ks, bool pk_two) {
    const int Hs = H >> up, Ws = W >> up;
#pragma unroll
    for (int i = 0; i < 5; ++i) {
        const int slot = (wi + 4 * i) * 64 + lane;
        const int blk = slot >> 4, res = slot & 15, cell = blk >> 3;
        const int ah = (cell / 3) * 4 + (res & 3), qh = (cell % 3) * 4 + (res >> 2);
        const int hf = blk & 1;
        const int ry = 2 * ah + ((blk >> 2) & 1), rx = 2 * qh + ((blk >> 1) & 1);
        const bool far = PACK && qh > pk_ks;
        const int y = y_in0 + ry, x = far ? rx - 2 * pk_ks - 3 : x_in0 + rx;
        const int qmax = (PACK && pk_ks < kTX) ? kTX + 1 : kTX;
        const bool iok = wi + 4 * i < kInPieces && ah <= kTY && qh <= qmax && y >= 0 && y < H && x >= 0 && x < W && (!far || pk_two);
        const size_t px = TR ? (size_t)(x >> up) * Hs + (y >> up) : (size_t)(y >> up) * Ws + (x >> up);
        ivo[i] = iok ? (unsigned)((px * Cs + 4 * hf) * sizeof(float)) +
                              (far ? (unsigned)((size_t)Hs * Ws * Cs * sizeof(float)) : 0u)
                        : 0u;
        imask[i] = __ballot(iok);
    }
}
#pragma clang diagnostic push
#pragma clang diagnostic ignored "-Winline-asm"
__device__ __forceinline__ void wino_issue_in(const float* buf, int wi, const unsigned (&ivo)[5], const unsigned long long (&imask)[5], const float* src) {
    unsigned long long sv_;
    const unsigned l0_ = lds_addr(buf + wi * 256);
    asm volatile("s_mov_b64 %0, exec\n"
                 "s_mov_b64 exec, %1\n s_mov_b32 m0, %6\n s_nop 0\n global_load_lds_dwordx4 %11, %16\n"
                 "s_mov_b64 exec, %2\n s_mov_b32 m0, %7\n s_nop 0\n global_load_lds_dwordx4 %12, %16\n"
                 "s_mov_b64 exec, %3\n s_mov_b32 m0, %8\n s_nop 0\n global_load_lds_dwordx4 %13, %16\n"
                 "s_mov_b64 exec, %4\n s_mov_b32 m0, %9\n s_nop 0\n global_load_lds_dwordx4 %14, %16\n"
                 "s_mov_b64 exec, %5\n s_mov_b32 m0, %10\n s_nop 0\n global_load_lds_dwordx4 %15, %16\n"
                 "s_mov_b64 exec, %0\n"
                 : "=&s"(sv_)
                 : "s"(imask[0]), "s"(imask[1]), "s"(imask[2]), "s"(imask[3]), "s"(imask[4]),
                   "s"(l0_), "s"(l0_ + 4096), "s"(l0_ + 8192), "s"(l0_ + 12288), "s"(l0_ + 16384),
                   "v"(ivo[0]), "v"(ivo[1]), "v"(ivo[2]), "v"(ivo[3]), "v"(ivo[4]), "s"(src)
                 : "memory", "m0");
}
#pragma clang diagnostic pop

constexpr int in_cs = 2 * 16 * 4;
constexpr int in_ms = 3 * 8 * 16 * 4;
template <bool PACK>
__device__ __forceinline__ float wino_frag(int (&in_a)[2], int (&in_b)[2], int wi, int li, int lh, int pk_ks) {
    const int tyl = li >> 3, txl = (li & 7) + ((PACK && (li & 7) >= pk_ks) ? 1 : 0);
    const int ra = (wi == 0) ? 0 : (wi == 2 ? 2 : 1);
    const int rb = (wi == 0) ? 2 : (wi == 1 ? 2 : (wi == 2 ? 1 : 3));
    auto unit = [&](int r, int ch) {
        const int ah = tyl + (r >> 1), qh = txl + ch;
        return ((((ah >> 2) * 3 + (qh >> 2)) * 8 + (r & 1) * 4 + lh) * 16 + 4 * (qh & 3) + (ah & 3)) * 4;
    };
    in_a[0] = unit(ra, 0); in_a[1] = unit(ra, 1);
    in_b[0] = unit(rb, 0); in_b[1] = unit(rb, 1);
    return (wi == 1) ? 1.f : -1.f;
}
__device__ __forceinline__ void wino_zero_ring(float* lds, int t, int nbuf, int y_in0, int x_in0, int H, int W, bool seam) {
    if (y_in0 < 0 || x_in0 < 0 || y_in0 + kRH > H || x_in0 + kRW > W || seam) {
        for (int i = t; i < nbuf * kInFloats / 4; i += 256) reinterpret_cast<f32x4*>(lds)[i] = f32x4{0.f, 0.f, 0.f, 0.f};
        asm volatile("s_waitcnt lgkmcnt(0)" ::: "memory");
        __syncthreads();
    }
}

struct WinoEpi { int H, W, Cout, relu, tbx, tby, pack_rx; };
template <bool PACK, bool FOLD, bool TR = false>
__device__ __forceinline__ void wino_output(float* lds, const f32x16 (&acc)[4][2][2], const ConvPtrs P, const WinoPatch pt, const WinoEpi e,
                                            const float inv_s, const float* btab, long long* dbg, const long long t_kend, const int t,
                                            const int wi) {
    const int H = e.H, W = e.W, Cout = e.Cout, HW = H * W;
    const int lane = PACK ? (int)__builtin_amdgcn_mbcnt_hi(~0u, __builtin_amdgcn_mbcnt_lo(~0u, 0u)) : t & 63;
    const int t_e = PACK ? wi * 64 + lane : t;
    const int oq = t_e & 15, otl = t_e >> 4;
    const bool o_far = PACK && (otl & 7) >= pt.pk_ks;
    const int ob = o_far ? pt.b + 1 : pt.b, otx = o_far ? (otl & 7) - pt.pk_ks : pt.tx0 + (otl & 7);
    const bool o_ok = !o_far || pt.pk_two;
    const int n = pt.nb * kBN + oq * 4;
    const f32x4 e_sc = (!FOLD && P.scale) ? *reinterpret_cast<const f32x4*>(P.scale + n) : f32x4{1.f, 1.f, 1.f, 1.f};
    const f32x4 e_sh = (!FOLD && P.shift) ? *reinterpret_cast<const f32x4*>(P.shift + n) : f32x4{0.f, 0.f, 0.f, 0.f};
    f32x4 e_res[4][4];
#pragma unroll
    for (int tp = 0; tp < 4; ++tp)
#pragma unroll
        for (int q = 0; q < 4; ++q) {
            const int ot = otl + 16 * tp;
            const int y = 2 * (pt.ty0 + (ot >> 3)) + (q >> 1), x = 2 * otx + (q & 1);
            e_res[tp][q] = (!FOLD && P.res && o_ok && y < H && x < W) ? *reinterpret_cast<const f32x4*>(P.res + ((size_t)ob * HW + (TR ? (size_t)x * H + y : (size_t)y * W + x)) * Cout + n)
                                                             : f32x4{0.f, 0.f, 0.f, 0.f};
        }
    __syncthreads();
    float* const zb = lds + ((wi * 2) * kNT + 4 * (lane >> 5)) * kBN + (lane & 31);
#pragma unroll
    for (int mt = 0; mt < 2; ++mt)
#pragma unroll
        for (int nt = 0; nt < 2; ++nt)
#pragma unroll
            for (int r = 0; r < 16; ++r) {
                const int mc = mt * 32 + (r & 3) + 8 * (r >> 2);
                const float m0 = acc[0][mt][nt][r], m1 = acc[1][mt][nt][r], m2 = acc[2][mt][nt][r], m3 = acc[3][mt][nt][r];
                zb[(0 * kNT + mc) * kBN + nt * 32] = m0 + m1 + m2;
                zb[(1 * kNT + mc) * kBN + nt * 32] = m1 - m2 - m3;
            }
    __syncthreads();
    f32x4 s1 = {0.f, 0.f, 0.f, 0.f}, s2 = {0.f, 0.f, 0.f, 0.f};
#pragma unroll
    for (int tp = 0; tp < 4; ++tp) {
        const int ot = otl + 16 * tp;
        const int oty = pt.ty0 + (ot >> 3);
        f32x4 z[4][2];
#pragma unroll
        for (int i = 0; i < 4; ++i)
#pragma unroll
            for (int cc = 0; cc < 2; ++cc) z[i][cc] = *reinterpret_cast<const f32x4*>(lds + ((i * 2 + cc) * kNT + ot) * kBN + oq * 4);
#pragma unroll
        for (int rr = 0; rr < 2; ++rr)
#pragma unroll
            for (int cc = 0; cc < 2; ++cc) {
                const int y = 2 * oty + rr, x = 2 * otx + cc;
                if (y >= H || x >= W || !o_ok) continue;
                f32x4 val = (rr == 0 ? z[0][cc] + z[1][cc] + z[2][cc] : z[1][cc] - z[2][cc] - z[3][cc]) * inv_s;
                if (FOLD) {
                    const int cls = (((y == 0) | ((y == H - 1) << 1)) << 2) | (x == 0) | ((x == W - 1) << 1);
                    val += *reinterpret_cast<const f32x4*>(btab + (size_t)cls * Cout + n);
                }
                if (!FOLD && P.scale) val = val * e_sc;
                val = val + e_sh;
                const size_t o = ((size_t)ob * HW + (TR ? (size_t)x * H + y : (size_t)y * W + x)) * Cout + n;
                if (!FOLD && P.res) val += e_res[tp][2 * rr + cc];
                if (!FOLD && e.relu) { val[0] = fmaxf(val[0], 0.f); val[1] = fmaxf(val[1], 0.f); val[2] = fmaxf(val[2], 0.f); val[3] = fmaxf(val[3], 0.f); }
                *reinterpret_cast<f32x4*>(P.out + o) = val;
                s1 += val;
                s2 += val * val;
            }
    }
    if (PACK && P.gn_part) {
        f32x4 q1[2] = {o_far ? f32x4{0.f, 0.f, 0.f, 0.f} : s1, o_far ? s1 : f32x4{0.f, 0.f, 0.f, 0.f}};
        f32x4 q2[2] = {o_far ? f32x4{0.f, 0.f, 0.f, 0.f} : s2, o_far ? s2 : f32x4{0.f, 0.f, 0.f, 0.f}};
#pragma unroll
        for (int sd = 0; sd < 2; ++sd)
#pragma unroll
            for (int o = 16; o < 64; o <<= 1)
#pragma unroll
                for (int k = 0; k < 4; ++k) { q1[sd][k] += __shfl_xor(q1[sd][k], o, 64); q2[sd][k] += __shfl_xor(q2[sd][k], o, 64); }
        __syncthreads();
        float* red = lds;
        if (lane < 16) {
#pragma unroll
            for (int sd = 0; sd < 2; ++sd)
#pragma unroll
                for (int k = 0; k < 4; ++k) {
                    red[((sd * 4 + wi) * kBN + oq * 4 + k) * 2] = q1[sd][k];
                    red[((sd * 4 + wi) * kBN + oq * 4 + k) * 2 + 1] = q2[sd][k];
                }
        }
        __syncthreads();
        if (t_e < 2 * kBN && (t_e < kBN || pt.pk_two)) {
            const int sd = t_e >> 6, ch = t_e & (kBN - 1);
            float u1 = 0.f, u2 = 0.f;
#pragma unroll
            for (int w = 0; w < 4; ++w) { u1 += red[((sd * 4 + w) * kBN + ch) * 2]; u2 += red[((sd * 4 + w) * kBN + ch) * 2 + 1]; }
            const int rx = e.pack_rx, Pn = e.tby * rx, slot = sd ? 0 : pt.pk_slot;
            float* g = P.gn_part + (((size_t)(pt.b + sd) * Pn + pt.by * rx + slot) * Cout + pt.nb * kBN + ch) * 2;
            g[0] = u1; g[1] = u2;
            if (sd == 0 && pt.pk_raw <= kTX)
                for (int z = slot + 1; z < rx; ++z) { g += (size_t)Cout * 2; g[0] = 0.f; g[1] = 0.f; }
        }
    } else if (P.gn_part) {
#pragma unroll
        for (int o = 16; o < 64; o <<= 1)
#pragma unroll
            for (int k = 0; k < 4; ++k) { s1[k] += __shfl_xor(s1[k], o, 64); s2[k] += __shfl_xor(s2[k], o, 64); }
        __syncthreads();
        float* red = lds;
        if (lane < 16) {
#pragma unroll
            for (int k = 0; k < 4; ++k) { red[(wi * kBN + oq * 4 + k) * 2] = s1[k]; red[(wi * kBN + oq * 4 + k) * 2 + 1] = s2[k]; }
        }
        __syncthreads();
        if (t_e < kBN) {
            float u1 = 0.f, u2 = 0.f;
#pragma unroll
            for (int w = 0; w < 4; ++w) { u1 += red[(w * kBN + t_e) * 2]; u2 += red[(w * kBN + t_e) * 2 + 1]; }
            const int Pn = e.tbx * e.tby;
            float* g = P.gn_part + (((size_t)pt.b * Pn + pt.by * e.tbx + pt.bx) * Cout + pt.nb * kBN + t_e) * 2;
            g[0] = u1; g[1] = u2;
        }
    }
    if (kWinoStamp && dbg && lane == 0) {
        asm volatile("s_waitcnt vmcnt(0)" ::: "memory");
        dbg[((size_t)blockIdx.x * 4 + wi) * 8 + 7] = clock64() - t_kend;
    }
}

inline int wino_tile_check(const WinoArgs& a, int groups, int kch, int step_bytes, bool packed, long long* nblk) {
    if (groups < 1 || groups > kMaxGroup || a.Cin % kch != 0 || a.Cout % kBN != 0 || (!kWinoStamp && a.dbg)) return FPC_EINVAL;
    if ((long long)a.H * a.W * a.Cin * (long long)sizeof(float) >= (1LL << 32)) return FPC_EINVAL;
    if ((long long)(a.Cin / kch) * step_bytes >= (1LL << 31)) return FPC_EINVAL;
    if (packed) {
        const WinoPackGeom q = wino_pack_geometry(a.H, a.W, a.B, a.Cin, a.orient ? a.pack > 1 : !a.fold);
        if (q.G != a.pack || q.tbx != a.tbx || q.tby != a.tby || q.rx != a.pack_rx) return FPC_EINVAL;
        *nblk = q.patches * (a.Cout / kBN) * groups;
    } else {
        if (a.tbx != cdiv(cdiv(a.W, 2), kTX) || a.tby != cdiv(cdiv(a.H, 2), kTY)) return FPC_EINVAL;
        *nblk = (long long)a.tbx * a.tby * a.B * (a.Cout / kBN) * groups;
    }
    return (*nblk < 1 || *nblk >= (1LL << 31)) ? FPC_EINVAL : 0;
}
}

int launch_wino_pack_fp16(const float* w_oihw, float* packed, int Cout, int Cin, bool pair, const float* w_also, int Cin_also, bool transpose,
                          hipStream_t s);

}
```

fastposecnn_amd/csrc/wino_w4.hip:

```cpp
#include <algorithm>
#ifdef FPC_STAMP_WINO
#include <cstdlib>
#endif
#include "wino_tile.hpp"

namespace fpc {
using namespace wino_tile;

typedef __bf16 bf16x8 __attribute__((ext_vector_type(8)));

namespace {
constexpr int kStepBytes = 12288 * 4;
static_assert(kLdsFloats >= 2 * kInFloats, "the K loop's two input buffers live in the output image's space");
}

template <int MODE>
__global__ __launch_bounds__(256, 1) void k_conv_wino_w4(const WinoArgs a) {
    __shared__ __attribute__((aligned(16))) float lds[kLdsFloats];
    long long* const dbg = kWinoStamp ? a.dbg : nullptr;
    const long long t_entry = dbg ? clock64() : 0;
    const int t = threadIdx.x, lane = t & 63;
    const int wi = __builtin_amdgcn_readfirstlane(t >> 6);
    const int li = lane & 31, lh = lane >> 5;
    const int H = a.H, W = a.W, Cin = a.Cin, Cout = a.Cout, HW = H * W;
    const int nkb = Cin >> 3;
    const WinoPatch pt = wino_patch<false>(blockIdx.x, Cout / kBN, a.groups, a.tbx, a.tby, 0, W, a.B);
    const int nb = pt.nb;
    const ConvPtrs P = wino_group(a.p[0], a.p[1], a.p[2], a.p[3], pt.grp);
    const int y_in0 = 2 * pt.ty0 - 1, x_in0 = 2 * pt.tx0 - 1;

    f32x16 acc[4][2][2];
    const __amdgpu_buffer_rsrc_t rs_w = make_rsrc(reinterpret_cast<const char*>(P.w) + (size_t)nb * nkb * kStepBytes);
    const int vo_u = li * 32 + 16 * (lh ^ ((li >> 3) & 1)), vo_t = li * 16 + 8 * (lh ^ ((li >> 4) & 1));
    int so_u = wi * 8192, so_t = 32768 + wi * 4096;
    u32x4 U[4][2];
    u32x2 T[4][2];
#define FPC_W4_LOAD_U(J, NT) U[J][NT] = __builtin_bit_cast(u32x4, __builtin_amdgcn_raw_buffer_load_b128(rs_w, vo_u, so_u + (J) * 2048 + (NT) * 1024, 0))
#define FPC_W4_LOAD_T(J, NT) T[J][NT] = __builtin_bit_cast(u32x2, __builtin_amdgcn_raw_buffer_load_b64(rs_w, vo_t, so_t + (J) * 1024 + (NT) * 512, 0))
#pragma unroll
    for (int j = 0; j < 4; ++j)
#pragma unroll
        for (int nt = 0; nt < 2; ++nt) { FPC_W4_LOAD_U(j, nt); FPC_W4_LOAD_T(j, nt); }
    if (nkb > 1) { so_u += kStepBytes; so_t += kStepBytes; }
    const float* isb = P.in + (size_t)pt.b * HW * Cin;
    unsigned ivo[5];
    unsigned long long imask[5];
    wino_stage_plan<false>(ivo, imask, wi, lane, y_in0, x_in0, H, W, Cin, 0, pt.pk_ks, pt.pk_two);
#define FPC_W4_ISSUE_IN(BUF) wino_issue_in(lds + (BUF) * kInFloats, wi, ivo, imask, isb)
    int in_a[2], in_b[2];
    const float sgn = wino_frag<false>(in_a, in_b, wi, li, lh, pt.pk_ks);
    wino_zero_ring(lds, t, 2, y_in0, x_in0, H, W, false);
    FPC_W4_ISSUE_IN(0);
    if (nkb > 1) isb += 8;
    FPC_W4_ISSUE_IN(1);
    if (nkb > 2) isb += 8;
#pragma unroll
    for (int j = 0; j < 4; ++j)
#pragma unroll
        for (int mt = 0; mt < 2; ++mt)
#pragma unroll
            for (int nt = 0; nt < 2; ++nt)
#pragma unroll
                for (int r = 0; r < 16; ++r) acc[j][mt][nt][r] = 0.f;

    asm volatile("s_waitcnt vmcnt(0)" ::: "memory");
    __syncthreads();

    u32x2 pa[4][2][3];
    f32x4 vn[2][4];
    {
#pragma unroll
        for (int mt = 0; mt < 2; ++mt) {
            f32x4 e[4];
#pragma unroll
            for (int c = 0; c < 4; ++c)
                e[c] = fma_s4(sgn, *reinterpret_cast<const f32x4*>(lds + in_b[c >> 1] + (c & 1) * in_cs + mt * in_ms),
                              *reinterpret_cast<const f32x4*>(lds + in_a[c >> 1] + (c & 1) * in_cs + mt * in_ms));
            vn[mt][0] = sub_s4(e[0], e[2]); vn[mt][1] = add_s4(e[1], e[2]); vn[mt][2] = sub_s4(e[2], e[1]); vn[mt][3] = sub_s4(e[1], e[3]);
#pragma unroll
            for (int j = 0; j < 3; ++j) split_bf3(vn[mt][j], pa[j][mt][0], pa[j][mt][1], pa[j][mt][2]);
        }
    }
    __syncthreads();

#define FPC_W4_MFMA(J, MT, NT, A, B) acc[J][MT][NT] = __builtin_amdgcn_mfma_f32_32x32x16_bf16(__builtin_bit_cast(bf16x8, A), __builtin_bit_cast(bf16x8, B), acc[J][MT][NT], 0, 0, 0)
#define FPC_W4_SPLIT_ITEM(J, MT, PART)                                                                        \
    do {                                                                                                      \
        const float x_ = vn[MT][J][PART];                                                                     \
        const unsigned xb_ = __builtin_bit_cast(unsigned, x_) & 0xFFFF0000u;                                  \
        const float r_ = x_ - __builtin_bit_cast(float, xb_);                                                 \
        const unsigned rb_ = __builtin_bit_cast(unsigned, r_) & 0xFFFF0000u;                                  \
        const float q_ = r_ - __builtin_bit_cast(float, rb_);                                                 \
        if ((PART) & 1) {                                                                                     \
            const unsigned k1_ = pack_hi16(sx[(PART) - 1], x_), k2_ = pack_hi16(sr[(PART) - 1], r_), k3_ = pack_hi16(sq[(PART) - 1], q_); \
            asm volatile("" :: "v"(k1_), "v"(k2_), "v"(k3_));                                                 \
            pa[J][MT][0][(PART) >> 1] = k1_; pa[J][MT][1][(PART) >> 1] = k2_; pa[J][MT][2][(PART) >> 1] = k3_; \
        } else {                                                                                              \
            asm volatile("" :: "v"(r_), "v"(q_));                                                             \
            sx[PART] = x_; sr[PART] = r_; sq[PART] = q_;                                                      \
        }                                                                                                     \
    } while (0)
#define FPC_W4_PIN4(V) asm volatile("" :: "v"(V))
    u32x4 Atup = {pa[0][0][0][0], pa[0][0][0][1], pa[0][0][0][0], pa[0][0][0][1]};
    int cur = 0;
    const long long c_begin = dbg ? clock64() : 0, r_begin = dbg ? wall_clock64() : 0;
#pragma unroll 1
    for (int kb = 0; kb < nkb; ++kb) {
        if (!(MODE & 2) && !(MODE & 8)) FPC_W4_ISSUE_IN(cur);
        const float* In = lds + (cur ^ 1) * kInFloats;
        f32x4 da[2][4], db[2][4], e[2][4];
        float sx[4], sr[4], sq[4];
        __builtin_amdgcn_s_setprio(1);
#pragma unroll
        for (int j = 0; j < 4; ++j) {
            u32x4 C[2];
#pragma unroll
            for (int g = 0; g < 3; ++g)
#pragma unroll
                for (int mt = 0; mt < 2; ++mt) {
                    const u32x4 Ause = Atup;
#pragma unroll
                    for (int nt = 0; nt < 2; ++nt) {
                        const int sl = 12 * j + 4 * g + 2 * mt + nt;
                        if (g < 2) FPC_W4_MFMA(j, mt, nt, Ause, U[j][nt]);
                        if (g == 1) {
                            if (mt == 0) C[nt] = u32x4{T[j][nt][0], T[j][nt][1], U[j][nt][0], U[j][nt][1]};
                            if (mt == 1 && !(MODE & 1)) FPC_W4_LOAD_U(j, nt);
                        }
                        if (g == 2) {
                            FPC_W4_MFMA(j, mt, nt, Ause, C[nt]);
                            if (mt == 1 && !(MODE & 1)) FPC_W4_LOAD_T(j, nt);
                        }
                        if (nt == 0) {
                            const int pr = (6 * j + 2 * g + mt + 1) % 24, nj = pr / 6, ng = (pr % 6) >> 1, nm = pr & 1;
                            const u32x2 lo = pa[nj][nm][ng == 1 ? 1 : 0], hi = pa[nj][nm][ng == 0 ? 0 : (ng == 1 ? 1 : 2)];
                            Atup = u32x4{lo[0], lo[1], hi[0], hi[1]};
                            FPC_W4_PIN4(Atup);
                        }
                        if (sl < 4) {
#pragma unroll
                            for (int c = 2 * (sl & 1); c < 2 * (sl & 1) + 2; ++c) {
                                da[sl >> 1][c] = *reinterpret_cast<const f32x4*>(In + in_a[c >> 1] + (c & 1) * in_cs + (sl >> 1) * in_ms);
                                db[sl >> 1][c] = *reinterpret_cast<const f32x4*>(In + in_b[c >> 1] + (c & 1) * in_cs + (sl >> 1) * in_ms);
                            }
                            FPC_W4_SPLIT_ITEM(3, 0, sl);
                        }
                        if (sl >= 4 && sl < 12) {
                            const int m_ = (sl - 4) >> 2, c = (sl - 4) & 3;
                            e[m_][c] = fma_s4(sgn, db[m_][c], da[m_][c]);
                            FPC_W4_PIN4(e[m_][c]);
                        }
                        if (sl >= 12 && sl < 16) FPC_W4_SPLIT_ITEM(3, 1, sl - 12);
                        if (sl >= 16 && sl < 24) {
                            const int m_ = (sl - 16) >> 2, jx = (sl - 16) & 3;
                            if (jx == 0) vn[m_][0] = sub_s4(e[m_][0], e[m_][2]);
                            if (jx == 1) vn[m_][1] = add_s4(e[m_][1], e[m_][2]);
                            if (jx == 2) vn[m_][2] = sub_s4(e[m_][2], e[m_][1]);
                            if (jx == 3) vn[m_][3] = sub_s4(e[m_][1], e[m_][3]);
                            FPC_W4_PIN4(vn[m_][jx]);
                        }
                        if (sl >= 24) {
                            const int q = (sl - 24) >> 2;
                            FPC_W4_SPLIT_ITEM(q >> 1, q & 1, (sl - 24) & 3);
                        }
                        __builtin_amdgcn_sched_barrier(0);
                    }
                }
        }
        __builtin_amdgcn_s_setprio(0);
        so_u += kb + 2 < nkb ? kStepBytes : 0;
        so_t += kb + 2 < nkb ? kStepBytes : 0;
        isb += kb + 3 < nkb ? 8 : 0;
        if (!(MODE & 2)) {
            if (MODE & 1) asm volatile("s_waitcnt vmcnt(0)" ::: "memory");
            else asm volatile("s_waitcnt vmcnt(16)" ::: "memory");
            if (!(MODE & 4)) __syncthreads();
        }
        cur ^= 1;
    }
#undef FPC_W4_MFMA
#undef FPC_W4_SPLIT_ITEM
#undef FPC_W4_PIN4
#undef FPC_W4_ISSUE_IN
#undef FPC_W4_LOAD_U
#undef FPC_W4_LOAD_T
    asm volatile("s_waitcnt vmcnt(0)" ::: "memory");
    const long long t_kend = dbg ? clock64() : 0;
    if (dbg && lane == 0) {
        long long* o = dbg + ((size_t)blockIdx.x * 4 + wi) * 8;
        o[0] = 0; o[1] = 0; o[2] = 0;
        o[3] = t_kend - c_begin; o[4] = wall_clock64() - r_begin; o[5] = nkb; o[6] = c_begin - t_entry;
    }
    wino_output<false, false>(lds, acc, P, pt, WinoEpi{H, W, Cout, a.relu, a.tbx, a.tby, 0}, 1.0f, nullptr, dbg, t_kend, t, wi);
}

int launch_conv_wino_w4(const WinoArgs& a, int groups, hipStream_t s) {
    long long nblk;
    if (const int rc = wino_tile_check(a, groups, 8, kStepBytes, false, &nblk)) return rc;
#ifdef FPC_STAMP_WINO
    static const int mode = getenv("FPC_W4_MODE") ? atoi(getenv("FPC_W4_MODE")) : 0;
    if (mode == 1) hipLaunchKernelGGL(k_conv_wino_w4<1>, dim3((unsigned)nblk), dim3(256), 0, s, a);
    else if (mode == 2) hipLaunchKernelGGL(k_conv_wino_w4<2>, dim3((unsigned)nblk), dim3(256), 0, s, a);
    else if (mode == 3) hipLaunchKernelGGL(k_conv_wino_w4<3>, dim3((unsigned)nblk), dim3(256), 0, s, a);
    else if (mode == 5) hipLaunchKernelGGL(k_conv_wino_w4<5>, dim3((unsigned)nblk), dim3(256), 0, s, a);
    else if (mode == 9) hipLaunchKernelGGL(k_conv_wino_w4<9>, dim3((unsigned)nblk), dim3(256), 0, s, a);
    else if (mode == 4) hipLaunchKernelGGL(k_conv_wino_w4<4>, dim3((unsigned)nblk), dim3(256), 0, s, a);
    else
#endif
    hipLaunchKernelGGL(k_conv_wino_w4<0>, dim3((unsigned)nblk), dim3(256), 0, s, a);
    return check_launch();
}

}
```

include/fpc.h:

```cpp
#ifndef FPC_H_
#define FPC_H_

#include <stddef.h>
#include <stdint.h>

#ifdef __cplusplus
extern "C" {
#endif

#define FPC_ABI_VERSION 11

#define FPC_OK 0
#define FPC_EINVAL (-1)
#define FPC_EWORKSPACE (-2)
#define FPC_ELAUNCH (-3)
#define FPC_EDEVICE (-4)
#define FPC_EFORMAT (-5)

typedef void* fpc_stream_t;

int fpc_abi_version(void);
const char* fpc_error_string(int code);
const char* fpc_last_hip_error(void);

int fpc_generate_hypothesis(const float* direct, const float* coords, const int32_t* idxs,
                            float* hyp, int tn, int vn, int hn, fpc_stream_t stream);

int fpc_voting_for_hypothesis(const float* direct, const float* coords, const float* hyp,
                              uint8_t* inliers, int tn, int vn, int hn, float inlier_thresh,
                              fpc_stream_t stream);

size_t fpc_ransac_workspace_bytes(int n, int H, int W, int hn);
int fpc_ransac_voting_v3(const float* mask, const float* vertex,
                         int64_t vs_n, int64_t vs_h, int64_t vs_w, int64_t vs_c,
                         int n, const int32_t* n_dev, int H, int W, int hn,
                         const int32_t* idxs, const uint8_t* keep, uint64_t seed,
                         float inlier_thresh, int min_num, int max_num,
                         float* out_xy, int32_t* out_tn, int32_t* out_win_idx,
                         int32_t* out_win_count, int32_t* out_inl_count,
                         float* out_hyp, int32_t* out_counts, double* out_refine,
                         void* ws, size_t ws_bytes, fpc_stream_t stream);
int fpc_ransac_voting_v3_bits(const float* mask, const uint64_t* mask_bits, const float* vertex,
                              int64_t vs_n, int64_t vs_h, int64_t vs_w, int64_t vs_c,
                              int n, const int32_t* n_dev, int H, int W, int hn,
                              const int32_t* idxs, const uint8_t* keep, uint64_t seed,
                              float inlier_thresh, int min_num, int max_num,
                              float* out_xy, int32_t* out_tn, int32_t* out_win_idx,
                              int32_t* out_win_count, int32_t* out_inl_count,
                              float* out_hyp, int32_t* out_counts, double* out_refine,
                              void* ws, size_t ws_bytes, fpc_stream_t stream);

int fpc_ransac_voting_v3_pose(const float* mask, const uint64_t* mask_bits, const float* vertex,
                              int64_t vs_n, int64_t vs_h, int64_t vs_w, int64_t vs_c,
                              int n, const int32_t* n_dev, int H, int W, int hn,
                              const int32_t* idxs, const uint8_t* keep, uint64_t seed,
                              float inlier_thresh, int min_num, int max_num,
                              float* out_xy, int32_t* out_tn, int32_t* out_win_idx,
                              int32_t* out_win_count, int32_t* out_inl_count,
                              float* out_hyp, int32_t* out_counts, double* out_refine,
                              const float* pose_q, const float* pose_z, const float* pose_kinv,
                              float* pose_R, float* pose_T, float* pose_RT,
                              void* ws, size_t ws_bytes, fpc_stream_t stream);

int fpc_vote_set_prune(int mode, int npass, const int32_t* cum16);
int fpc_vote_prune_info(const void* ws, size_t ws_bytes, int n, int H, int W, int hn, int32_t* out, fpc_stream_t stream);

int fpc_class_compress(const float* mask_logits, const float* quat, const float* scales,
                       const float* xy, const float* z, const int64_t* cat_mask_in,
                       int B, int C, int HW,
                       int64_t* cat_mask, float* oq, float* os, float* oxy, float* oz,
                       fpc_stream_t stream);
int fpc_class_compress_bits(const float* mask_logits, const float* quat, const float* scales,
                            const float* xy, const float* z, const int64_t* cat_mask_in,
                            int B, int C, int HW,
                            int64_t* cat_mask, float* oq, float* os, float* oxy, float* oz,
                            uint64_t* fg_bits, fpc_stream_t stream);


size_t fpc_cc_workspace_bytes(int B, int H, int W);
int fpc_cc_label(const int64_t* cat_mask, int B, int H, int W,
                 int32_t* labels, int32_t* n_out, int32_t* root_pix, int cap,
                 void* ws, size_t ws_bytes, fpc_stream_t stream);
int fpc_cc_bits_supported(int B, int H, int W);
int fpc_fg_bits(const int64_t* cat_mask, int B, int H, int W, uint64_t* fg_bits, fpc_stream_t stream);
int fpc_cc_label_bits(const uint64_t* fg_bits, int B, int H, int W, int32_t* labels, int32_t* n_out,
                      int32_t* root_pix, int cap, void* ws, size_t ws_bytes, fpc_stream_t stream);


size_t fpc_aggregate_workspace_bytes(int N);
int fpc_aggregate(const int32_t* labels, const int64_t* cat_mask,
                  const float* quat, const float* scales, const float* xy, const float* z,
                  int B, int H, int W, int N, const int32_t* n_dev,
                  int64_t* class_ids, int64_t* sample_ids, float* inst_masks,
                  float* oq, float* os, float* oz, float* oxy, float* out_stats,
                  void* ws, size_t ws_bytes, fpc_stream_t stream);
size_t fpc_mask_bits_words(int H, int W);
int fpc_aggregate_bits(const int32_t* labels, const int64_t* cat_mask,
                       const float* quat, const float* scales, const float* xy, const float* z,
                       int B, int H, int W, int N, const int32_t* n_dev,
                       int64_t* class_ids, int64_t* sample_ids, float* inst_masks,
                       float* oq, float* os, float* oz, float* oxy, float* out_stats, uint64_t* inst_bits,
                       const int32_t* root_pix, void* ws, size_t ws_bytes, fpc_stream_t stream);

int fpc_pose_rt(const float* q, const float* xy, const float* z, const float* kinv, int n,
                float* R, float* T, float* RT, fpc_stream_t stream);

int fpc_pack_pose_records(const int64_t* sample_ids, const int64_t* class_ids, const float* q, const float* scales,
                          const float* xy, const float* z, const float* R, const float* T, const float* RT, int n,
                          int sample_offset, int capacity, float* out, fpc_stream_t stream);

size_t fpc_mask_iou_workspace_bytes(int n1, int n2, int64_t hw);
int fpc_mask_iou(const void* masks1, int n1, const void* masks2, int n2, int64_t hw, int elem_size,
                 float* iou, int32_t* inter, int32_t* uni, void* ws, size_t ws_bytes, fpc_stream_t stream);

size_t fpc_preprocess_workspace_bytes(int B);
int fpc_preprocess_u8(const uint8_t* img_hwc, int B, int H, int W, const double* mean3, const double* std3,
                      int input_range_01, float* out_nchw, void* ws, size_t ws_bytes, fpc_stream_t stream);

int fpc_png_info(const uint8_t* data, size_t nbytes, int32_t* out5);
int fpc_png_decode(const uint8_t* data, size_t nbytes, void* out, size_t out_bytes, int mode);
int fpc_png_decode_batch(const uint8_t* const* datas, const size_t* sizes, int n, uint8_t* out, int H, int W, int threads);

int fpc_gt_build(const uint8_t* ids, int64_t pix_stride, int64_t frame_stride, int B, int H, int W,
                 const int16_t* row_of, const uint8_t* class_of, const int32_t* first_row, int n,
                 int64_t* class_mask, void* inst_masks, int mask_elem, int32_t* pix_count, fpc_stream_t stream);
int fpc_depth_decode(const void* src, int src_kind, int channels, int B, int H, int W, float* depth_f32, fpc_stream_t stream);

int fpc_pose_errors(const float* q0, const float* q1, const int64_t* symmetric_ids, const float* rot, int nrot,
                    const float* RT1, const float* RT2, const float* scales1, const float* scales2,
                    const float* T1, const float* T2, int n, double* out_degree, float* out_iou3d, float* out_offset,
                    fpc_stream_t stream);

size_t fpc_pose_metrics_state_words(int num_classes, int n_deg, int n_iou, int n_off, int n_complex);
int fpc_pose_metrics_update(const int32_t* order, const int32_t* match_pred, const int32_t* count, int n1, int n2,
                            const float* gt_quaternion, const float* gt_RT, const float* gt_scales, const float* gt_T,
                            const int64_t* symmetric_ids, const int64_t* class_ids, const float* quaternion, const float* RT,
                            const float* scales, const float* T, const float* rot, int nrot, const double* thr_degree, int n_deg,
                            const double* thr_iou, int n_iou, const double* thr_offset, int n_off, const double* thr_complex,
                            int n_complex, const double* thr_table, int num_classes, int64_t* state, double* raw_degree,
                            float* raw_iou, float* raw_offset, int32_t* raw_class, int raw_capacity, fpc_stream_t stream);

int fpc_confusion_update(const int64_t* pred, const int64_t* gt, int64_t n, int num_classes, int64_t* state, fpc_stream_t stream);

int fpc_post_network_backward(const int32_t* labels, const float* cat_xy, int B, int H, int W, int N,
                              const int32_t* n_dev, const double* table, float inlier_thresh, int max_num,
                              uint64_t seed, const uint8_t* keep, float* g_q, float* g_s, float* g_xy, float* g_z,
                              fpc_stream_t stream);
int fpc_vote_refine_backward(const float* mask, const float* vertex, int64_t vs_n, int64_t vs_h, int64_t vs_w,
                             int64_t vs_c, int n, int H, int W, const double* table, float inlier_thresh, int max_num,
                             uint64_t seed, const uint8_t* keep, float* g_vertex, fpc_stream_t stream);
int fpc_class_compress_backward(const int64_t* cat_mask, const float* quat, const float* xy, const float* go_q,
                                const float* go_s, const float* go_xy, const float* go_z, int B, int C, int HW,
                                float* g_q, float* g_s, float* g_xy, float* g_z, fpc_stream_t stream);
int fpc_mask_losses(const float* logits, const int64_t* target, int B, int C, int HW, int64_t ignore_ce,
                    int64_t ignore_cce, float alpha, float gamma, double* sums6, const float* w3, float* grad,
                    fpc_stream_t stream);
#define FPC_MATCH_MAX_INSTANCES 1024
int fpc_match_assign(const float* iou, const int64_t* gt_cls, const int64_t* pred_cls, int n1, int n2, int32_t* match_pred,
                     int32_t* order, int32_t* count, fpc_stream_t stream);
#define FPC_LOSS_L2 0
#define FPC_LOSS_L1 1
#define FPC_LOSS_SMOOTH_L1 2
int fpc_matched_losses(const int32_t* order, const int32_t* match_pred, const int32_t* count, int n1, int n2,
                       const float* gt_quaternion, const float* gt_xy, const float* gt_z, const float* gt_scales,
                       const int64_t* symmetric_ids, const float* quaternion, const float* xy, const float* z,
                       const float* scales, const float* rot, int nrot, double eps, int xy_type, int z_type, int scales_type,
                       const double* weights, double* losses, double* task_total, double* matched_total, int32_t* best_rot,
                       fpc_stream_t stream);
int fpc_matched_losses_backward(const int32_t* order, const int32_t* match_pred, const int32_t* count, int n1, int n2,
                                const float* gt_quaternion, const float* gt_xy, const float* gt_z, const float* gt_scales,
                                const int64_t* symmetric_ids, const float* quaternion, const float* xy, const float* z,
                                const float* scales, const float* rot, int nrot, double eps, int xy_type, int z_type,
                                int scales_type, const double* weights, const double* losses, const int32_t* best_rot,
                                const double* g_losses, float* g_quaternion, float* g_xy, float* g_z, float* g_scales,
                                fpc_stream_t stream);
int fpc_grad_sumsq(const float* g, size_t n, double* out2, fpc_stream_t stream);
int fpc_lookahead_radam_step(float* p, const float* g, float* m, float* v, float* slow, size_t n, float lr, float beta1,
                             float beta2, float eps, float weight_decay, int64_t step, int la_k, float la_alpha,
                             const float* ctl, fpc_stream_t stream);

typedef struct fpc_net fpc_net_t;
int fpc_net_create(const char* encoder, int classes, int B, int H, int W, fpc_net_t** out);
int fpc_net_create_encoder(int block, const int* layers4, int classes, int B, int H, int W, fpc_net_t** out);
void fpc_net_destroy(fpc_net_t* net);
int fpc_net_param_count(const fpc_net_t* net);
const char* fpc_net_param_name(const fpc_net_t* net, int i);
int64_t fpc_net_param_numel(const fpc_net_t* net, int i);
size_t fpc_net_workspace_bytes(const fpc_net_t* net);
int fpc_net_load_params(fpc_net_t* net, const float* const* params, int count, void* ws, size_t ws_bytes,
                        fpc_stream_t stream);
int fpc_net_forward(fpc_net_t* net, const float* x, float* logits_mask, float* logits_quat,
                    float* logits_scales, float* logits_xy, float* logits_z, int64_t* cat_mask,
                    float* cq, float* cs, float* cxy, float* cz, fpc_stream_t stream);
int fpc_net_forward_bits(fpc_net_t* net, const float* x, float* logits_mask, float* logits_quat,
                         float* logits_scales, float* logits_xy, float* logits_z, int64_t* cat_mask,
                         float* cq, float* cs, float* cxy, float* cz, uint64_t* fg_bits, fpc_stream_t stream);

int fpc_net_autotune_next(fpc_net_t* net, int mode );
int fpc_net_set_split_precision(fpc_net_t* net, int on);
int fpc_net_set_graph(fpc_net_t* net, int on);
int fpc_net_graph_recorded(const fpc_net_t* net);
int fpc_net_conv_count(const fpc_net_t* net);
int fpc_net_conv_plan(const fpc_net_t* net, int i, int* out5);
int fpc_net_copy_plans(fpc_net_t* dst, const fpc_net_t* src);
int fpc_net_force_winograd(fpc_net_t* net, int form);
int fpc_net_force_pointwise(fpc_net_t* net, int on);
int fpc_net_force_fold(fpc_net_t* net, int on);
int fpc_net_force_direct_h3(fpc_net_t* net, int on);
int fpc_net_force_stem_pool(fpc_net_t* net, int on);
int fpc_act_range(const float* x, long long n, unsigned* rec4, fpc_stream_t stream);
int fpc_net_survey_next(fpc_net_t* net, unsigned* records_dev, int sites);
int fpc_net_guard_ranges(fpc_net_t* net, const unsigned* records_host, int sites, float lo, float hi);
int fpc_net_guarded(const fpc_net_t* net, int i);
int fpc_stem_pool_tasks(int Ho, int Wo, int64_t* out4);
int fpc_wino_pack_geometry(int H, int W, int B, int Cin, int fold, int64_t* out8);
int fpc_net_set_wino_pack(fpc_net_t* net, int on);
int fpc_net_set_wino_orient(fpc_net_t* net, int on);
int fpc_wino_orient_geometry(int H, int W, int B, int Cin, int fold, int pack, int64_t* out9);
int64_t fpc_net_wino_blocks(const fpc_net_t* net);
int fpc_net_flops(const fpc_net_t* net, double* out3);
int fpc_net_tensor(const fpc_net_t* net, const char* name, const float** ptr, int* H, int* W, int* C);

enum {
    FPC_PLAN_WINO_ORIENT = -11, FPC_PLAN_WINO_PACKED = -10, FPC_PLAN_TWO_LAUNCH = 100, FPC_PLAN_BF3 = 1000, FPC_PLAN_LATERAL = 2000, FPC_PLAN_STEM = 3000,
    FPC_PLAN_STEM_POOL = 3100, FPC_PLAN_POINTWISE = 4000, FPC_PLAN_FOLDED = 5000, FPC_PLAN_H3 = 6000, FPC_PLAN_LATERAL_H3 = 7000
};
size_t fpc_conv2d_workspace_bytes(int B, int Ho, int Wo, int Cin, int Cout, int Kh, int Kw);
size_t fpc_conv2d_workspace_bytes_for(int B, int Ho, int Wo, int Cin, int Cout, int Kh, int Kw, int bm, int bn, int nsplit);
int fpc_conv2d_plan(int B, int Ho, int Wo, int Cin, int Cout, int Kh, int Kw, int bm, int bn, int nsplit,
                    int* out4 );
int fpc_conv2d(const float* in, int64_t sb, int64_t sh, int64_t sw, int64_t sc, const float* w_oihw,
               const float* scale, const float* shift, const float* res, const float* up, float* out,
               float* gn_part, int B, int Hi, int Wi, int Cin, int Cout, int Kh, int Kw, int stride, int pad,
               int relu, int bm, int bn, int nsplit, void* ws, size_t ws_bytes, fpc_stream_t stream);

size_t fpc_conv2d_wgrad_workspace_bytes(int B, int Ho, int Wo, int Cin, int Cout, int Kh, int Kw);
int fpc_conv2d_wgrad(const float* x, int64_t sb, int64_t sh, int64_t sw, const float* dy, float* dw, int B, int Hi,
                     int Wi, int Cin, int Cout, int Kh, int Kw, int stride, int pad, void* ws, size_t ws_bytes,
                     fpc_stream_t stream);
int fpc_conv2d_wgrad_split(const float* x, int64_t sb, int64_t sh, int64_t sw, const float* dy, float* dw, int B, int Hi,
                           int Wi, int Cin, int Cout, int Kh, int Kw, int stride, int pad, void* ws, size_t ws_bytes,
                           fpc_stream_t stream);

int fpc_upsample_bilinear_fwd(const float* in, int64_t sb, int64_t sc, int64_t sh, int64_t sw, float* out, int B, int C, int h,
                              int w, int scale, int out_nhwc, fpc_stream_t stream);
size_t fpc_upsample_bilinear_bwd_scratch_floats(int B, int C, int h, int w, int scale);
int fpc_upsample_bilinear_bwd(const float* dout, int64_t sb, int64_t sc, int64_t sh, int64_t sw, float* din, float* scratch,
                              int B, int C, int h, int w, int scale, int din_nhwc, fpc_stream_t stream);

size_t fpc_groupnorm4_relu_scratch_floats(int B, int HW, int C);
int fpc_groupnorm4_relu_fwd(const float* x, const float* gamma, const float* beta, float* y, float* stats, float* part, int B,
                            int HW, int C, int groups, float eps, fpc_stream_t stream);
int fpc_groupnorm4_relu_bwd(const float* x, const float* dy, const float* gamma, const float* beta, const float* stats, float* dx,
                            float* part, int B, int HW, int C, int groups, fpc_stream_t stream);

size_t fpc_batchnorm_scratch_floats(int P, int C);
int fpc_batchnorm_fwd(const float* x, const float* res, const float* gamma, const float* beta, float* running_mean,
                      float* running_var, float* y, float* stats, float* part, int P, int C, float eps, float momentum, int relu,
                      fpc_stream_t stream);
int fpc_batchnorm_bwd(const float* x, const float* y, const float* dy, const float* gamma, const float* stats, float* dx,
                      float* dres, float* dgamma, float* dbeta, float* part, int P, int C, int relu, fpc_stream_t stream);

#ifdef __cplusplus
}
#endif
#endif
```

Baseline: 2780.

## Use reciprocal-multiply block decode and addtid LDS stores in Winograd epilogue

Replaces integer divides and modulos in the Winograd block-index decode with precomputed magic-multiply reciprocals computed on the host and passed in the kernel args. Rewrites the Winograd output Z-tile staging into LDS as batched ds_write_addtid_b32 inline asm with a new run-based LDS layout, and updates the matching read addressing. It also adds stamp-only timing probes and test and AB tooling. The asm path depends on exact offset reach and m0 setup, and the LDS footprint grows slightly.

```diff
diff --git a/fastposecnn_amd/_native.py b/fastposecnn_amd/_native.py
--- a/fastposecnn_amd/_native.py
+++ b/fastposecnn_amd/_native.py
@@ -97,6 +97,8 @@
     "fpc_net_set_wino_pack": (_i, [_vp, _i]),
     "fpc_net_set_wino_orient": (_i, [_vp, _i]),
     "fpc_wino_orient_geometry": (_i, [_i, _i, _i, _i, _i, _i, ctypes.POINTER(_i64)]),
+    "fpc_wino_recip": (_i, [ctypes.c_uint32, ctypes.POINTER(_i64)]),
+    "fpc_wino_decode": (_i, [_i, _i, _i, _i, _i, _i, _i, ctypes.POINTER(_i64)]),
     "fpc_net_wino_blocks": (_i64, [_vp]),
     "fpc_net_graph_recorded": (_i, [_vp]),
     "fpc_net_flops": (_i, [_vp, ctypes.POINTER(ctypes.c_double)]),
diff --git a/fastposecnn_amd/csrc/net.hip b/fastposecnn_amd/csrc/net.hip
--- a/fastposecnn_amd/csrc/net.hip
+++ b/fastposecnn_amd/csrc/net.hip
@@ -1444,6 +1444,20 @@
     return FPC_OK;
 }
 
+extern "C" int fpc_wino_recip(uint32_t d, int64_t* out2) {
+    if (!out2 || d < 1 || d > (1u << 31)) return FPC_EINVAL;
+    const WinoRecip r = wino_recip(d);
+    out2[0] = r.m; out2[1] = r.sh;
+    return FPC_OK;
+}
+extern "C" int fpc_wino_decode(int Cout, int groups, int tbx, int tby, int W, int B, int pack, int64_t* out14) {
+    if (!out14 || Cout < 64 || groups < 1 || tbx < 1 || tby < 1 || W < 1 || B < 1 || pack < 0) return FPC_EINVAL;
+    const WinoDecode d = wino_decode(Cout, groups, tbx, tby, W, B, pack);
+    const WinoRecip r[7] = {d.nnb, d.groups, d.tbx, d.tby, d.per, d.tbxl, d.tcw};
+    for (int i = 0; i < 7; ++i) { out14[2 * i] = r[i].m; out14[2 * i + 1] = r[i].sh; }
+    return FPC_OK;
+}
+
 extern "C" size_t fpc_conv2d_workspace_bytes(int B, int Ho, int Wo, int Cin, int Cout, int Kh, int Kw) {
     int K = Cin * Kh * Kw, Kpad = cdiv(K, kConvBK) * kConvBK, Npad = cdiv(Cout, kConvNAlign) * kConvNAlign;
     size_t packed = conv_packed_floats(Npad, Kpad);
diff --git a/fastposecnn_amd/csrc/net_kernels.hpp b/fastposecnn_amd/csrc/net_kernels.hpp
--- a/fastposecnn_amd/csrc/net_kernels.hpp
+++ b/fastposecnn_amd/csrc/net_kernels.hpp
@@ -164,6 +164,21 @@
 #else
 constexpr bool kWinoStamp = false;
 #endif
+constexpr int kWinoSerialStamps = 16;
+
+struct WinoRecip { unsigned m; int sh; };
+inline WinoRecip wino_recip(unsigned d) {
+    int l = 0;
+    while ((1ull << l) < d) ++l;
+    const int sh = 31 + l;
+    return WinoRecip{(unsigned)(((1ull << sh) + d - 1) / d), sh};
+}
+struct WinoDecode { WinoRecip nnb, groups, tbx, tby, per, tbxl, tcw; };
+inline WinoDecode wino_decode(int Cout, int groups, int tbx, int tby, int W, int B, int pack) {
+    const int tcw = (W + 1) / 2, last = pack > 0 ? ((B % pack) * tcw + 7) / 8 : 0;
+    return WinoDecode{wino_recip(Cout / 64), wino_recip(groups), wino_recip(tbx), wino_recip(tby), wino_recip(tbx * tby),
+                      wino_recip(last ? last : tbx), wino_recip(tcw)};
+}
 
 struct WinoArgs {
     ConvPtrs p[kMaxGroup];
@@ -179,6 +194,7 @@
     int fold, Cin2;
     int pack, pack_rx;
     int orient;
+    WinoDecode dec;
 };
 int launch_conv_wino(const WinoArgs& a, int groups, hipStream_t s);
 const float* zero_page();
diff --git a/fastposecnn_amd/csrc/wino_h2.hip b/fastposecnn_amd/csrc/wino_h2.hip
--- a/fastposecnn_amd/csrc/wino_h2.hip
+++ b/fastposecnn_amd/csrc/wino_h2.hip
@@ -22,7 +22,7 @@
     const int li = lane & 31, lh = lane >> 5;
     const int H = a.H, W = a.W, Cin = a.Cin, Cout = a.Cout, HW = H * W;
     const int nkb = Cin >> 3;
-    const WinoPatch pt = wino_patch<false>(blockIdx.x, Cout / kBN, a.groups, a.tbx, a.tby, 0, W, a.B);
+    const WinoPatch pt = wino_patch<false>(blockIdx.x, Cout / kBN, a.groups, a.tbx, a.tby, 0, W, a.B, a.dec);
     const int nb = pt.nb, nnb = Cout / kBN;
     const ConvPtrs P = wino_group(a.p[0], a.p[1], a.p[2], a.p[3], pt.grp);
     const int y_in0 = 2 * pt.ty0 - 1, x_in0 = 2 * pt.tx0 - 1;
@@ -264,9 +264,11 @@
     return launch_wino_pack_fp16(w_oihw, packed, Cout, Cin, false, nullptr, 0, false, s);
 }
 
-int launch_conv_wino_h2(const WinoArgs& a, int groups, hipStream_t s) {
+int launch_conv_wino_h2(const WinoArgs& a_in, int groups, hipStream_t s) {
     long long nblk;
-    if (const int rc = wino_tile_check(a, groups, 8, kStepBytes, false, &nblk)) return rc;
+    if (const int rc = wino_tile_check(a_in, groups, 8, kStepBytes, false, &nblk)) return rc;
+    WinoArgs a = a_in;
+    a.dec = wino_decode(a.Cout, groups, a.tbx, a.tby, a.W, a.B, 0);
 #ifdef FPC_STAMP_WINO
     static const int mode = getenv("FPC_H2_MODE") ? atoi(getenv("FPC_H2_MODE")) : 0;
     if (mode == 1) hipLaunchKernelGGL(k_conv_wino_h2<1>, dim3((unsigned)nblk), dim3(256), 0, s, a);
diff --git a/fastposecnn_amd/csrc/wino_h3.hip b/fastposecnn_amd/csrc/wino_h3.hip
--- a/fastposecnn_amd/csrc/wino_h3.hip
+++ b/fastposecnn_amd/csrc/wino_h3.hip
@@ -31,10 +31,12 @@
     const int li = lane & 31, lh = lane >> 5;
     const int H = a.H, W = a.W, Cout = a.Cout;
     const int nnb = Cout / kBN;
-    const WinoPatch pt = wino_patch<PACK>(blockIdx.x, nnb, a.groups, a.tbx, a.tby, a.pack, W, a.B);
+    const WinoPatch pt = wino_patch<PACK>(blockIdx.x, nnb, a.groups, a.tbx, a.tby, a.pack, W, a.B, a.dec);
     const int nb = pt.nb, grp = pt.grp, pk_ks = pt.pk_ks;
     const ConvPtrs P = wino_group(a.p[0], a.p[1], a.p[2], a.p[3], grp);
     const int y_in0 = 2 * pt.ty0 - 1, x_in0 = 2 * pt.tx0 - 1;
+    const bool fine = kWinoStamp && dbg && a.variant == kWinoSerialStamps;
+    long long t_dec = fine ? clock64() : 0, t_wld = 0, t_plan = 0, t_zero = 0;
 
     f32x16 acc[4][2][2];
     float inv_s = 1.f;
@@ -61,6 +63,7 @@
 #pragma unroll
         for (int nt = 0; nt < 2; ++nt) { FPC_H3_LOAD_U1(j, nt); FPC_H3_LOAD_U2(j, nt); }
     if (npair > 1) so_u += kPairBytes;
+    if (PH == 0) t_wld = fine ? clock64() : 0;
 
     const float* isb = sgpr_ptr(src + (size_t)pt.b * (H >> up) * (W >> up) * Cs);
     unsigned ivo[5];
@@ -69,7 +72,9 @@
 #define FPC_H3_ISSUE_IN(BUF, PTR) wino_issue_in(lds + (BUF) * kInFloats, wi, ivo, imask, PTR)
     int in_a[2], in_b[2];
     const float sgn = wino_frag<PACK>(in_a, in_b, wi, li, lh, pk_ks);
+    if (PH == 0) t_plan = fine ? clock64() : 0;
     wino_zero_ring(lds, t, kRing, y_in0, x_in0, H, W, PACK && pk_ks < kTX);
+    if (PH == 0) t_zero = fine ? clock64() : 0;
     FPC_H3_ISSUE_IN(0, isb);
     isb += 8;
     FPC_H3_ISSUE_IN(1, isb);
@@ -243,8 +248,10 @@
         o[0] = t_issued - t_entry; o[1] = t_landed - t_issued; o[2] = t_synced - t_landed;
         o[3] = t_kend - c_begin; o[4] = wall_clock64() - r_begin; o[5] = a.Cin >> 3; o[6] = c_begin - t_entry;
     }
+    long long* const fdbg = (!(FOLD && PACK) && fine) ? dbg + (size_t)gridDim.x * 32 + ((size_t)blockIdx.x * 4 + wi) * 16 : nullptr;
+    if (fdbg && lane == 0) { fdbg[0] = t_dec - t_entry; fdbg[1] = t_wld - t_entry; fdbg[2] = t_plan - t_entry; fdbg[3] = t_zero - t_entry; fdbg[4] = t_issued - t_entry; }
     wino_output<PACK, FOLD, TR>(lds, acc, P, pt, WinoEpi{H, W, Cout, a.relu, a.tbx, a.tby, a.pack_rx}, inv_s,
-                            wino_group(a.btab[0], a.btab[1], a.btab[2], a.btab[3], grp), dbg, t_kend, t, wi);
+                            wino_group(a.btab[0], a.btab[1], a.btab[2], a.btab[3], grp), dbg, t_kend, t, wi, fdbg);
 }
 
 WinoPackGeom wino_pack_geometry(int H, int W, int B, int Cin, bool allow) {
@@ -291,13 +298,15 @@
     return *transposed ? wino_pack_geometry(W, H, B, Cin, !g1) : wino_pack_geometry(H, W, B, Cin, pack_allow);
 }
 
-int launch_conv_wino_h3(const WinoArgs& a, int groups, hipStream_t s) {
+int launch_conv_wino_h3(const WinoArgs& a_in, int groups, hipStream_t s) {
     long long nblk;
-    if (a.orient) {
+    if (a_in.orient) {
+        const WinoArgs& a = a_in;
         WinoArgs t = a;
         std::swap(t.H, t.W);
         if (a.pack < 1 || a.dbg) return FPC_EINVAL;
         if (const int rc = wino_tile_check(t, groups, 16, kPairBytes, true, &nblk)) return rc;
+        t.dec = wino_decode(t.Cout, groups, t.tbx, t.tby, t.W, t.B, t.pack);
         if (a.fold) {
             if (const int rc = wino_fold_check(a, groups)) return rc;
             hipLaunchKernelGGL((k_conv_wino_h3<0, true, true, true>), dim3((unsigned)nblk), dim3(256), 0, s, t);
@@ -306,7 +315,9 @@
         }
         return check_launch();
     }
-    if (const int rc = wino_tile_check(a, groups, 16, kPairBytes, a.pack > 1, &nblk)) return rc;
+    if (const int rc = wino_tile_check(a_in, groups, 16, kPairBytes, a_in.pack > 1, &nblk)) return rc;
+    WinoArgs a = a_in;
+    a.dec = wino_decode(a.Cout, groups, a.tbx, a.tby, a.W, a.B, a.pack > 1 ? a.pack : 0);
     if (a.pack > 1) {
         hipLaunchKernelGGL((k_conv_wino_h3<0, false, true>), dim3((unsigned)nblk), dim3(256), 0, s, a);
         return check_launch();
@@ -318,6 +329,8 @@
     }
 #ifdef FPC_STAMP_WINO
     static const int var = getenv("FPC_H3_VAR") ? atoi(getenv("FPC_H3_VAR")) : 0;
+    static const bool serial = getenv("FPC_WINO_SERIAL") && atoi(getenv("FPC_WINO_SERIAL")) != 0;
+    if (serial && a.dbg) a.variant = kWinoSerialStamps;
     if (var == 1) hipLaunchKernelGGL((k_conv_wino_h3<1, false, false>), dim3((unsigned)nblk), dim3(256), 0, s, a);
     else
 #endif
diff --git a/fastposecnn_amd/csrc/wino_tile.hpp b/fastposecnn_amd/csrc/wino_tile.hpp
--- a/fastposecnn_amd/csrc/wino_tile.hpp
+++ b/fastposecnn_amd/csrc/wino_tile.hpp
@@ -17,7 +17,13 @@
 constexpr int kInPieces = 18;
 constexpr int kInFloats = kInPieces * 256;
 constexpr int kPairBytes = 16 * 2 * 2 * 64 * 16;
-constexpr int kLdsFloats = 4 * 2 * kNT * kBN;
+constexpr int kZOdd = 64 * 1024 + 128;
+constexpr int z_run(int cc, int mt, int r, int nt) { return ((((cc * 2 + mt) * 8 + (r >> 1)) * 2 + nt) * 4) * 256 + (r & 1) * kZOdd; }
+constexpr int kZOddM0 = 64704;
+constexpr int kZM0Slack = 65535 - 3 * 256 - kZOddM0;
+static_assert(z_run(1, 1, 15, 1) - kZOddM0 < 65536 && z_run(0, 0, 1, 0) >= kZOddM0 && kZM0Slack >= 0, "ds_write_addtid_b32's reach");
+constexpr int kLdsFloats = 4 * 2 * kNT * kBN + 32;
+static_assert(z_run(1, 1, 15, 1) + 3 * 256 + 256 == kLdsFloats * 4, "the last run ends the image");
 
 __device__ __forceinline__ __amdgpu_buffer_rsrc_t make_rsrc(const void* base) {
     return __builtin_amdgcn_make_buffer_rsrc(const_cast<void*>(base), 0, 0x7FFFFFFF, 0x00020000);
@@ -35,24 +41,28 @@
     int pk_ks, pk_raw, pk_slot;
     bool pk_two;
 };
+__device__ __forceinline__ int wino_div(int n, const WinoRecip r) { return (int)(((unsigned long long)(unsigned)n * r.m) >> r.sh); }
 template <bool PACK>
-__device__ __forceinline__ WinoPatch wino_patch(int bid, int nnb, int groups, int tbx, int tby, int pack, int W, int B) {
+__device__ __forceinline__ WinoPatch wino_patch(int bid, int nnb, int groups, int tbx, int tby, int pack, int W, int B, const WinoDecode dc) {
     WinoPatch q;
     q.pk_ks = 99; q.pk_raw = 99; q.pk_slot = 0; q.pk_two = false;
-    q.nb = bid % nnb; bid /= nnb;
-    q.grp = bid % groups; bid /= groups;
+    int up = wino_div(bid, dc.nnb);
+    q.nb = bid - up * nnb; bid = up;
+    up = wino_div(bid, dc.groups);
+    q.grp = bid - up * groups; bid = up;
     if constexpr (!PACK) {
-        q.bx = bid % tbx; bid /= tbx;
-        q.by = bid % tby;
-        q.b = bid / tby;
+        up = wino_div(bid, dc.tbx);
+        q.bx = bid - up * tbx; bid = up;
+        q.b = wino_div(bid, dc.tby);
+        q.by = bid - q.b * tby;
         q.tx0 = q.bx * kTX;
     } else {
         const int G = pack, tcw = (W + 1) >> 1, per = tbx * tby;
-        const int g = bid / per, rem = bid - g * per;
+        const int g = wino_div(bid, dc.per), rem = bid - g * per;
         const int nf = min(G, B - g * G);
         const int tbxg = min(tbx, (nf * tcw + kTX - 1) / kTX);
-        q.bx = rem % tbxg; q.by = rem / tbxg;
-        const int f = (kTX * q.bx) / tcw;
+        q.by = wino_div(rem, tbxg == tbx ? dc.tbx : dc.tbxl); q.bx = rem - q.by * tbxg;
+        const int f = wino_div(kTX * q.bx, dc.tcw);
         q.tx0 = kTX * q.bx - f * tcw;
         q.b = g * G + f;
         q.pk_raw = tcw - q.tx0;
@@ -138,10 +148,12 @@
 }
 
 struct WinoEpi { int H, W, Cout, relu, tbx, tby, pack_rx; };
+#pragma clang diagnostic push
+#pragma clang diagnostic ignored "-Winline-asm"
 template <bool PACK, bool FOLD, bool TR = false>
 __device__ __forceinline__ void wino_output(float* lds, const f32x16 (&acc)[4][2][2], const ConvPtrs P, const WinoPatch pt, const WinoEpi e,
                                             const float inv_s, const float* btab, long long* dbg, const long long t_kend, const int t,
-                                            const int wi) {
+                                            const int wi, long long* fdbg = nullptr) {
     const int H = e.H, W = e.W, Cout = e.Cout, HW = H * W;
     const int lane = PACK ? (int)__builtin_amdgcn_mbcnt_hi(~0u, __builtin_amdgcn_mbcnt_lo(~0u, 0u)) : t & 63;
     const int t_e = PACK ? wi * 64 + lane : t;
@@ -163,20 +175,44 @@
                                                              : f32x4{0.f, 0.f, 0.f, 0.f};
         }
     __syncthreads();
-    float* const zb = lds + ((wi * 2) * kNT + 4 * (lane >> 5)) * kBN + (lane & 31);
-#pragma unroll
-    for (int mt = 0; mt < 2; ++mt)
-#pragma unroll
-        for (int nt = 0; nt < 2; ++nt)
-#pragma unroll
-            for (int r = 0; r < 16; ++r) {
-                const int mc = mt * 32 + (r & 3) + 8 * (r >> 2);
-                const float m0 = acc[0][mt][nt][r], m1 = acc[1][mt][nt][r], m2 = acc[2][mt][nt][r], m3 = acc[3][mt][nt][r];
-                zb[(0 * kNT + mc) * kBN + nt * 32] = m0 + m1 + m2;
-                zb[(1 * kNT + mc) * kBN + nt * 32] = m1 - m2 - m3;
-            }
+    if (kWinoStamp && fdbg && (t & 63) == 0) fdbg[8] = clock64() - t_kend;
+    {
+        const unsigned zm0 = lds_addr(lds) + wi * 256;
+#pragma unroll
+        for (int mt = 0; mt < 2; ++mt)
+#pragma unroll
+            for (int nt = 0; nt < 2; ++nt)
+#pragma unroll
+                for (int cc = 0; cc < 2; ++cc)
+#pragma unroll
+                    for (int odd = 0; odd < 2; ++odd) {
+                        float z[8];
+#pragma unroll
+                        for (int h = 0; h < 8; ++h) {
+                            const int r = 2 * h + odd;
+                            const float m0 = acc[0][mt][nt][r], m1 = acc[1][mt][nt][r], m2 = acc[2][mt][nt][r], m3 = acc[3][mt][nt][r];
+                            z[h] = cc == 0 ? m0 + m1 + m2 : m1 - m2 - m3;
+                        }
+#define FPC_Z_IMM(H) "i"(z_run(cc, mt, 2 * (H) + odd, nt) - odd * kZOddM0)
+                        asm volatile("s_mov_b32 m0, %8\n s_nop 0\n"
+                                     "ds_write_addtid_b32 %0 offset:%9\n ds_write_addtid_b32 %1 offset:%10\n"
+                                     "ds_write_addtid_b32 %2 offset:%11\n ds_write_addtid_b32 %3 offset:%12\n"
+                                     "ds_write_addtid_b32 %4 offset:%13\n ds_write_addtid_b32 %5 offset:%14\n"
+                                     "ds_write_addtid_b32 %6 offset:%15\n ds_write_addtid_b32 %7 offset:%16\n"
+                                     :: "v"(z[0]), "v"(z[1]), "v"(z[2]), "v"(z[3]), "v"(z[4]), "v"(z[5]), "v"(z[6]), "v"(z[7]),
+                                        "s"(zm0 + odd * kZOddM0), FPC_Z_IMM(0), FPC_Z_IMM(1), FPC_Z_IMM(2), FPC_Z_IMM(3), FPC_Z_IMM(4),
+                                        FPC_Z_IMM(5), FPC_Z_IMM(6), FPC_Z_IMM(7)
+                                     : "memory", "m0");
+#undef FPC_Z_IMM
+                    }
+        asm volatile("s_waitcnt lgkmcnt(0)" ::: "memory");
+    }
+    if (kWinoStamp && fdbg && (t & 63) == 0) fdbg[9] = clock64() - t_kend;
     __syncthreads();
+    if (kWinoStamp && fdbg && (t & 63) == 0) fdbg[10] = clock64() - t_kend;
     f32x4 s1 = {0.f, 0.f, 0.f, 0.f}, s2 = {0.f, 0.f, 0.f, 0.f};
+    const float* const zr = lds + z_run(0, 0, (otl & 3) + 4 * (otl >> 3), oq >> 3) / 4 +
+                            ((otl >> 2) & 1) * 32 + (oq & 7) * 4;
 #pragma unroll
     for (int tp = 0; tp < 4; ++tp) {
         const int ot = otl + 16 * tp;
@@ -185,7 +221,7 @@
 #pragma unroll
         for (int i = 0; i < 4; ++i)
 #pragma unroll
-            for (int cc = 0; cc < 2; ++cc) z[i][cc] = *reinterpret_cast<const f32x4*>(lds + ((i * 2 + cc) * kNT + ot) * kBN + oq * 4);
+            for (int cc = 0; cc < 2; ++cc) z[i][cc] = *reinterpret_cast<const f32x4*>(zr + (z_run(cc, tp >> 1, 8 * (tp & 1), 0) + 256 * i) / 4);
 #pragma unroll
         for (int rr = 0; rr < 2; ++rr)
 #pragma unroll
@@ -207,6 +243,7 @@
                 s2 += val * val;
             }
     }
+    if (kWinoStamp && fdbg && (t & 63) == 0) fdbg[11] = clock64() - t_kend;
     if (PACK && P.gn_part) {
         f32x4 q1[2] = {o_far ? f32x4{0.f, 0.f, 0.f, 0.f} : s1, o_far ? s1 : f32x4{0.f, 0.f, 0.f, 0.f}};
         f32x4 q2[2] = {o_far ? f32x4{0.f, 0.f, 0.f, 0.f} : s2, o_far ? s2 : f32x4{0.f, 0.f, 0.f, 0.f}};
@@ -260,11 +297,13 @@
             g[0] = u1; g[1] = u2;
         }
     }
+    if (kWinoStamp && fdbg && lane == 0) fdbg[12] = clock64() - t_kend;
     if (kWinoStamp && dbg && lane == 0) {
         asm volatile("s_waitcnt vmcnt(0)" ::: "memory");
         dbg[((size_t)blockIdx.x * 4 + wi) * 8 + 7] = clock64() - t_kend;
     }
 }
+#pragma clang diagnostic pop
 
 inline int wino_tile_check(const WinoArgs& a, int groups, int kch, int step_bytes, bool packed, long long* nblk) {
     if (groups < 1 || groups > kMaxGroup || a.Cin % kch != 0 || a.Cout % kBN != 0 || (!kWinoStamp && a.dbg)) return FPC_EINVAL;
diff --git a/fastposecnn_amd/csrc/wino_w4.hip b/fastposecnn_amd/csrc/wino_w4.hip
--- a/fastposecnn_amd/csrc/wino_w4.hip
+++ b/fastposecnn_amd/csrc/wino_w4.hip
@@ -24,7 +24,7 @@
     const int li = lane & 31, lh = lane >> 5;
     const int H = a.H, W = a.W, Cin = a.Cin, Cout = a.Cout, HW = H * W;
     const int nkb = Cin >> 3;
-    const WinoPatch pt = wino_patch<false>(blockIdx.x, Cout / kBN, a.groups, a.tbx, a.tby, 0, W, a.B);
+    const WinoPatch pt = wino_patch<false>(blockIdx.x, Cout / kBN, a.groups, a.tbx, a.tby, 0, W, a.B, a.dec);
     const int nb = pt.nb;
     const ConvPtrs P = wino_group(a.p[0], a.p[1], a.p[2], a.p[3], pt.grp);
     const int y_in0 = 2 * pt.ty0 - 1, x_in0 = 2 * pt.tx0 - 1;
@@ -194,9 +194,11 @@
     wino_output<false, false>(lds, acc, P, pt, WinoEpi{H, W, Cout, a.relu, a.tbx, a.tby, 0}, 1.0f, nullptr, dbg, t_kend, t, wi);
 }
 
-int launch_conv_wino_w4(const WinoArgs& a, int groups, hipStream_t s) {
+int launch_conv_wino_w4(const WinoArgs& a_in, int groups, hipStream_t s) {
     long long nblk;
-    if (const int rc = wino_tile_check(a, groups, 8, kStepBytes, false, &nblk)) return rc;
+    if (const int rc = wino_tile_check(a_in, groups, 8, kStepBytes, false, &nblk)) return rc;
+    WinoArgs a = a_in;
+    a.dec = wino_decode(a.Cout, groups, a.tbx, a.tby, a.W, a.B, 0);
 #ifdef FPC_STAMP_WINO
     static const int mode = getenv("FPC_W4_MODE") ? atoi(getenv("FPC_W4_MODE")) : 0;
     if (mode == 1) hipLaunchKernelGGL(k_conv_wino_w4<1>, dim3((unsigned)nblk), dim3(256), 0, s, a);
diff --git a/include/fpc.h b/include/fpc.h
--- a/include/fpc.h
+++ b/include/fpc.h
@@ -217,6 +217,8 @@
 int fpc_net_set_wino_pack(fpc_net_t* net, int on);
 int fpc_net_set_wino_orient(fpc_net_t* net, int on);
 int fpc_wino_orient_geometry(int H, int W, int B, int Cin, int fold, int pack, int64_t* out9);
+int fpc_wino_recip(uint32_t d, int64_t* out2);
+int fpc_wino_decode(int Cout, int groups, int tbx, int tby, int W, int B, int pack, int64_t* out14);
 int64_t fpc_net_wino_blocks(const fpc_net_t* net);
 int fpc_net_flops(const fpc_net_t* net, double* out3);
 int fpc_net_tensor(const fpc_net_t* net, const char* name, const float** ptr, int* H, int* W, int* C);
diff --git a/tools_dev/wino_serial_digest.py b/tools_dev/wino_serial_digest.py
--- /dev/null
+++ b/tools_dev/wino_serial_digest.py
@@ -0,0 +1,113 @@
+import functools
+import hashlib
+import json
+import os
+import sys
+
+ROOT = os.path.dirname(os.path.dirname(os.path.abspath(__file__)))
+sys.path.insert(0, ROOT)
+sys.path.insert(0, os.path.join(ROOT, "tests"))
+import torch
+
+REQUESTS = (-7, -8, -9, -10, -11)
+SHAPES = [(B, H, W) for H, W in ((24, 32), (23, 31)) for B in (2, 3, 5)] + [(2, 40, 24), (3, 40, 24)]
+COUTS = (64, 128)
+EPILOGUES = ("none", "bn_relu_res", "gn")
+FOLD_B = (2, 3)
+FOLD_HW = (96, 128)
+
+
+def cins(request):
+    return (16, 32, 48) if request <= -9 else (16, 48)
+
+
+def conv_cases(request):
+    return [(f"r{request}-b{B}-{Cin}x{H}x{W}-{Cout}-{epi}", request, B, Cin, H, W, Cout, epi)
+            for B, H, W in SHAPES for Cin in cins(request) for Cout in COUTS for epi in EPILOGUES]
+
+
+@functools.lru_cache(maxsize=None)
+def operands(B, Cin, H, W, Cout):
+    g = torch.Generator().manual_seed(((B * 64 + Cin) * 64 + H) * 256 + W * 2 + Cout // 128)
+    x = torch.randn((B, Cin, H, W), generator=g)
+    w = torch.randn((Cout, Cin, 3, 3), generator=g) / (Cin * 9) ** 0.5
+    scale, shift = torch.rand(Cout, generator=g) + 0.5, torch.randn(Cout, generator=g)
+    res = torch.randn((B, Cout, H, W), generator=g)
+    return x, w, scale, shift, res
+
+
+def epilogue_args(epi, scale, shift, res):
+    if epi == "bn_relu_res":
+        return scale, shift, res, True, False
+    return None, None, None, False, epi == "gn"
+
+
+def run_conv(dev, request, x, w, scale=None, shift=None, res=None, relu=False, gn=False):
+    from test_gpu_wino_pack import _conv
+    t = lambda a: None if a is None else a.contiguous().to(dev)
+    out, gp, _ = _conv(dev, x.permute(0, 2, 3, 1).contiguous().to(dev), w.contiguous().to(dev), request, scale=t(scale), shift=t(shift),
+                       res=None if res is None else res.permute(0, 2, 3, 1).contiguous().to(dev), relu=relu, gn=gn)
+    return out.cpu(), None if gp is None else gp.cpu()
+
+
+def run_case(dev, case):
+    _, request, B, Cin, H, W, Cout, epi = case
+    x, w, scale, shift, res = operands(B, Cin, H, W, Cout)
+    s, h, r, relu, gn = epilogue_args(epi, scale, shift, res)
+    return run_conv(dev, request, x, w, scale=s, shift=h, res=r, relu=relu, gn=gn)
+
+
+def fold_engine(dev, B):
+    import fastposecnn_amd.lib as L
+    from fastposecnn_amd.engine import NetEngine
+    from test_gpu_p2_fold import _model
+    m, _ = _model(L)
+    m = m.to(dev)
+    eng = NetEngine(m, B, FOLD_HW[0], FOLD_HW[1], dev, autotune=False, split_precision=3)
+    eng.force_winograd(9)
+    eng.force_fold(1)
+    assert any(p[2] == 5000 for p in eng.conv_plans()), "s2.0 is not folded"
+    return m, eng
+
+
+def run_fold(dev, B, orient, built=None):
+    from fastposecnn_amd import synth
+    m, eng = built or fold_engine(dev, B)
+    eng.set_wino_orient(orient)
+    x = torch.stack([synth.make_image(i, *FOLD_HW) for i in range(B)]).to(dev)
+    with torch.no_grad():
+        logits, _ = eng.forward(x)
+    torch.cuda.synchronize()
+    out = {f"fold-b{B}-orient{orient}-d{d}.seg6": eng.tensor(f"d{d}.seg6").detach().cpu().clone() for d in range(4)}
+    out.update({f"fold-b{B}-orient{orient}-logits.{k}": v.detach().cpu().clone() for k, v in sorted(logits.items())})
+    return out
+
+
+def digest(t):
+    return hashlib.sha256(t.contiguous().numpy().tobytes()).hexdigest()
+
+
+def case_digests(dev, case):
+    out, gp = run_case(dev, case)
+    d = {case[0] + ":out": digest(out)}
+    if gp is not None:
+        d[case[0] + ":records"] = digest(gp)
+    return d
+
+
+def main():
+    dev = torch.device("cuda:0")
+    d = {}
+    for request in REQUESTS:
+        for case in conv_cases(request):
+            d.update(case_digests(dev, case))
+    for B in FOLD_B:
+        built = fold_engine(dev, B)
+        for orient in (1, 0):
+            d.update({k: digest(v) for k, v in run_fold(dev, B, orient, built).items()})
+    json.dump(d, sys.stdout, indent=0, sort_keys=True)
+    print()
+
+
+if __name__ == "__main__":
+    main()
diff --git a/tools_dev/wino_serial_site_ab.py b/tools_dev/wino_serial_site_ab.py
--- /dev/null
+++ b/tools_dev/wino_serial_site_ab.py
@@ -0,0 +1,64 @@
+import csv, os, statistics, sys
+
+SHAPES = [("layer1", 32, 64, 120, 160, 64), ("s2.0-unfolded", 32, 256, 120, 160, 128), ("layer2", 32, 128, 60, 80, 128), ("s3.0", 32, 256, 60, 80, 128)]
+WARM, N = 3, 10
+
+
+def run(root):
+    sys.path.insert(0, os.path.abspath(root))
+    import torch
+    from fastposecnn_amd import _native as nat
+    dev = torch.device("cuda:0")
+    L = nat.lib()
+    for name, B, Cin, H, W, Cout in SHAPES:
+        g = torch.Generator().manual_seed(Cin + H)
+        x = torch.randn((B, H, W, Cin), generator=g).to(dev)
+        w = (torch.randn((Cout, Cin, 3, 3), generator=g) * 0.05).to(dev)
+        out = torch.empty((B, H, W, Cout), device=dev)
+        ws = torch.empty(L.fpc_conv2d_workspace_bytes(B, H, W, Cin, Cout, 3, 3), dtype=torch.uint8, device=dev)
+        sb, sh, sw, sc = x.stride()
+        st = torch.cuda.current_stream().cuda_stream
+        for i in range(WARM + N):
+            for ns in (-9, -11):
+                nat.check(L.fpc_conv2d(x.data_ptr(), sb, sh, sw, sc, w.data_ptr(), None, None, None, None, out.data_ptr(), None, B, H, W, Cin,
+                                       Cout, 3, 3, 1, 1, 0, 0, 0, ns, ws.data_ptr(), ws.numel(), st), "conv")
+            torch.cuda.synchronize()
+    print("done")
+
+
+def times(path):
+    rows = [r for r in csv.DictReader(open(path)) if "k_conv_wino_h3" in r["Kernel_Name"]]
+    rows.sort(key=lambda r: int(r["Start_Timestamp"]))
+    per = 2 * (WARM + N)
+    assert len(rows) == per * len(SHAPES), (path, len(rows))
+    out = {}
+    for si in range(len(SHAPES)):
+        blk = rows[si * per:(si + 1) * per]
+        for v in (0, 1):
+            out[(si, v)] = [(int(r["End_Timestamp"]) - int(r["Start_Timestamp"])) / 1e3 for r in blk[2 * WARM + v::2]]
+    return out
+
+
+def parse(args):
+    sides = {}
+    for a in args:
+        tag, paths = a.split("=")
+        acc = {}
+        for p in paths.split(","):
+            for k, v in times(p).items():
+                acc.setdefault(k, []).extend(v)
+        sides[tag] = acc
+    (ta, A), (tb, Bv) = list(sides.items())
+    for si, s in enumerate(SHAPES):
+        for v, rq in enumerate((-9, -11)):
+            a, b = A[(si, v)], Bv[(si, v)]
+            ma, mb = statistics.median(a), statistics.median(b)
+            print("%-14s %dx%dx%dx%d->%d request %3d  %s %8.1f us (%.1f-%.1f, n=%d) | %s %8.1f us (%.1f-%.1f, n=%d) | %+.2f %%"
+                  % (s[0], s[1], s[2], s[3], s[4], s[5], rq, ta, ma, min(a), max(a), len(a), tb, mb, min(b), max(b), len(b), 100 * (mb / ma - 1)))
+
+
+if __name__ == "__main__":
+    if sys.argv[1] == "run":
+        run(sys.argv[2])
+    else:
+        parse(sys.argv[2:])
diff --git a/tools_dev/wino_serial_stamps.py b/tools_dev/wino_serial_stamps.py
--- /dev/null
+++ b/tools_dev/wino_serial_stamps.py
@@ -0,0 +1,29 @@
+import os, sys
+os.environ["FPC_WINO_SERIAL"] = "1"
+sys.path.insert(0, os.path.dirname(os.path.dirname(os.path.abspath(__file__))))
+import torch
+from fastposecnn_amd import _native as nat
+dev = torch.device("cuda:0"); L = nat.lib()
+if not hasattr(L, "fpc_dbg_wino_diag"):
+    sys.exit("wino_serial_stamps.py needs a diagnostic build of the library (build.build(extra=['-DFPC_STAMP_WINO']))")
+B, Cin, Hi, Wi, Cout = (int(v) for v in sys.argv[1:6])
+x = torch.randn((B, Hi, Wi, Cin), device=dev); w = torch.randn((Cout, Cin, 3, 3), device=dev) * 0.05
+out = torch.empty((B, Hi, Wi, Cout), device=dev)
+ws = torch.empty(L.fpc_conv2d_workspace_bytes(B, Hi, Wi, Cin, Cout, 3, 3), dtype=torch.uint8, device=dev)
+nblk = -(-(-(-Wi // 2)) // 8) * -(-(-(-Hi // 2)) // 8) * B * (Cout // 64)
+dbg = torch.zeros((nblk * 4 * (8 + 16),), dtype=torch.int64, device=dev)
+sb, sh, sw, sc = x.stride(); st = torch.cuda.current_stream().cuda_stream
+for _ in range(50):
+    nat.check(L.fpc_conv2d(x.data_ptr(), sb, sh, sw, sc, w.data_ptr(), None, None, None, None, out.data_ptr(), dbg.data_ptr(), B, Hi, Wi,
+                           Cin, Cout, 3, 3, 1, 1, 77, 0, 0, -9, ws.data_ptr(), ws.numel(), st), "conv")
+torch.cuda.synchronize()
+d = dbg.cpu().double()
+a = d[:nblk * 32].view(nblk, 4, 8); f = d[nblk * 32:].view(nblk, 4, 16)
+assert (f[:, :, 4] > 0).all(), "no serial-path records: is this the plain -9 launch of a diagnostic build?"
+m = lambda t: t.mean().item()
+issued = a[:, :, 0]; landed = issued + a[:, :, 1]; synced = landed + a[:, :, 2]
+print("shape %d x %d x %d x %d -> %d: clock %.0f MHz, K loop %.0f ticks" % (B, Cin, Hi, Wi, Cout, m(a[:, :, 3] / a[:, :, 4] * 100.0), m(a[:, :, 3])))
+print("  entry: decode %.0f | weights requested %.0f | plan %.0f | ring zeroed %.0f | issued, acc zeroed %.0f (%.0f) | landed %.0f | barrier %.0f | loop %.0f"
+      % (m(f[:, :, 0]), m(f[:, :, 1]), m(f[:, :, 2]), m(f[:, :, 3]), m(f[:, :, 4]), m(issued), m(landed), m(synced), m(a[:, :, 6])))
+print("  exit:  barrier %.0f | Z stores %.0f | barrier %.0f | reads, epilogue, last store %.0f | records %.0f | acknowledged %.0f"
+      % (m(f[:, :, 8]), m(f[:, :, 9]), m(f[:, :, 10]), m(f[:, :, 11]), m(f[:, :, 12]), m(a[:, :, 7])))
```

Result: faster. 2812 (median of 6 runs) (+1.1%).
